# Chriz122/ultralytics_pro

Measured on AMD Instinct MI355X. Metric: images/sec (whole job = n_gpus x per-GPU bs=32) YOLOv8n 640x640 (forward + Detect decode + NMS), higher is better.
Workload: dtype bf16

## Files before the change

### include/upa.h

```cpp
#ifndef UPA_H
#define UPA_H
#include <stddef.h>
#include <stdint.h>

#ifdef __cplusplus
extern "C" {
#endif

enum { UPA_F32 = 0, UPA_BF16 = 1, UPA_U8_BGR_HWC = 2  };
enum { UPA_ACT_NONE = 0, UPA_ACT_SILU = 1, UPA_ACT_RELU = 2 };
enum { UPA_OK = 0, UPA_EINVAL = -1, UPA_EUNSUPPORTED = -2, UPA_EWORKSPACE = -3, UPA_ELAUNCH = -4 };

typedef struct upa_opts {
  uint32_t size;
  int32_t conv_big;
  int32_t conv_big_bm;
  int32_t conv_ckt;
  int32_t no_ws, no_pipe, no_1x1, no_c16, no_upcat;
  int32_t pipe_all;
  int32_t pipe_min_tiles;
  int32_t pipe_wgs, c16_wgs;
  int32_t c1_mt, c1_waves, c1_wgs;
  int32_t pair;
  int32_t pair_tile64, pair_tile32;
  int32_t no_pair_cv2;
  int32_t c2f;
  int32_t c2f16_waves;
  int32_t c2f32_th;
  int32_t no_branch_tail;
  int32_t branch_tail_bm;
  int32_t stem_wgs, stemf_wgs, stemf_waves, stem_no_mfma;
  int32_t ablate_conv, ablate_pipe, ablate_c1, ablate_stem;
  int32_t c2f64_max_px;
  int32_t conv_ws3;
  int32_t no_group;
  int32_t no_c2f32_up;
  int32_t no_xcd;
  int32_t keys_only;
  int32_t conv_p8;
  int32_t c2f_stream;
  int32_t c2f_stream_rows;
  int32_t no_stack_first;
  int32_t no_epi_stats;
  int32_t nms_stages;
  int32_t nms_first_prefix;
  int32_t detect_stream;
  int32_t detect_stream_rows;
  int32_t no_sppf_front;
  int32_t no_c2f16_down;
} upa_opts;

int upa_version(void);
const char* upa_last_error(void);
size_t upa_opts_size(void);

size_t upa_conv_packed_weight_bytes(int cout, int cin, int k, int dtype);
int upa_pack_conv_weight(const float* w_oihw, int cout, int cin, int k, int dtype, void* out);
int upa_conv2d_bias_act(const void* x, int n, int h, int w, int cin, int ldx,
                        const void* w_packed, const float* bias ,
                        void* y, int cout, int ldy,
                        const void* residual , int ldr,
                        int k, int stride, int pad, int act, int dtype, const upa_opts* opts, void* stream);
typedef struct upa_conv_problem {
  const void* x; int32_t n, h, w, cin, ldx;
  const void* w_packed; const float* bias;
  void* y; int32_t cout, ldy;
  const void* residual; int32_t ldr;
} upa_conv_problem;
int upa_conv2d_bias_act_group(const upa_conv_problem* probs, int count, int k, int stride, int pad, int act, int dtype,
                              const upa_opts* opts, void* stream);

int upa_conv2d_pool2(const void* x, int n, int h, int w, int cin, int ldx, const void* w_packed, const float* bias, void* y, int cout,
                     int ldy, int k, int stride, int pad, int act, int dtype, const upa_opts* opts, void* stream);
int upa_conv2d_stem_nchw_pool2(const void* x_nchw, int x_dtype, int n, int cin, int h, int w, const float* w_oihw, const float* bias,
                               void* y, int cout, int ldy, int k, int stride, int pad, int act, int dtype, const upa_opts* opts,
                               void* stream);

int upa_conv_variant(int n, int h, int w, int cin, int cout, int k, int stride, int pad, int dtype, const upa_opts* opts);

int upa_bottleneck_pair(const void* x, int n, int h, int w, int c, int ldx, const void* w1_packed, const float* b1,
                        const void* w2_packed, const float* b2, void* y, int ldy, int residual, int act, int dtype,
                        const upa_opts* opts, void* stream);
int upa_bottleneck_pair_e(const void* x, int n, int h, int w, int c, int cmid, int ldx, const void* w1_packed, const float* b1,
                          const void* w2_packed, const float* b2, void* y, int ldy, int residual, int act, int dtype,
                          const upa_opts* opts, void* stream);


size_t upa_stem_packed_weight_bytes(int cout, int cin, int k);
int upa_pack_stem_weight(const float* w_oihw, int cout, int cin, int k, float* out );
int upa_conv2d_stem_nchw(const void* x_nchw, int x_dtype, int n, int cin, int h, int w,
                         const float* w_oihw, const float* bias, void* y, int cout, int ldy,
                         int k, int stride, int pad, int act, int dtype, const upa_opts* opts, void* stream);

int upa_stem_conv_fused(const void* x, int n, int h, int w, const float* w0, const float* b0, const void* w1,
                        const float* b1, void* y, int ldy, const upa_opts* opts, void* stream);
int upa_stem_conv_fused_k(const void* x, int n, int h, int w, int k0, const float* w0, const float* b0, const void* w1,
                          const float* b1, void* y, int ldy, const upa_opts* opts, void* stream);
int upa_stem_conv_fused_c(const void* x, int n, int h, int w, int k0, int c0, const float* w0, const float* b0, const void* w1,
                          const float* b1, void* y, int ldy, const upa_opts* opts, void* stream);
int upa_stem_conv_fused_s(const void* x, int n, int h, int w, int k0, int s0, int c0, const float* w0, const float* b0,
                          const void* w1, const float* b1, void* y, int ldy, const upa_opts* opts, void* stream);

int upa_maxpool2d(const void* x, int n, int h, int w, int c, int ldx, void* y, int oh, int ow, int ldy,
                  int k, int stride, int pad, int pad_br, int dtype, void* stream);
int upa_sppf_pool3(const void* x, int n, int h, int w, int c, int ldx, void* y1, void* y2, void* y3, int ldy,
                   int dtype, void* stream);
int upa_sppf_front(const void* x, int n, int h, int w, int c1, int ldx, const void* w_packed, const float* bias, void* y, int c_, int ldy, int dtype,
                   const upa_opts* opts, void* stream);
int upa_upsample2x(const void* x, int n, int h, int w, int c, int ldx, void* y, int ldy, int dtype, void* stream);
int upa_copy_view(const void* x, int n, int h, int w, int c, int ldx, void* y, int ldy, int dtype, void* stream);
int upa_copy_to_host(const void* src_dev, void* dst_pinned, size_t bytes, void* stream);
int upa_results_to_host(const void* rows_dev, const int* counts_dev, int batch, int max_rows, int row_bytes,
                        void* rows_pinned, int* counts_pinned, void* stream);
int upa_add_view(const void* a, int lda, const void* b, int ldb, void* y, int ldy, int n, int h, int w, int c,
                 int dtype, void* stream);
int upa_nchw_to_nhwc(const float* x, int n, int c, int h, int w, void* y, int ldy, int dtype, void* stream);
int upa_nhwc_to_nchw(const void* x, int n, int h, int w, int c, int ldx, float* y, int dtype, void* stream);
int upa_letterbox_u8(const void* src, int n, int h0, int w0, long src_image_stride, int src_row_stride, void* dst, int H, int W,
                     int new_h, int new_w, int top, int left, int pad_value, void* stream);


int upa_detect_decode(const void* box, int ldb, const void* cls, int ldc, int n, int h, int w, int reg_max, int nc,
                      float stride_px, float* y, int a_total, int a0, int dtype, void* stream);
int upa_detect_tail(const void* x, int n, int h, int w, int cin, int ldx, const void* w_packed, const float* bias, int cout,
                    int kind, int nc, float stride_px, float* y, int a_total, int a0, void* raw, int ldraw,
                    unsigned long long* best_keys, int dtype, const upa_opts* opts, void* stream);

int upa_conv1x1_upcat(const void* x, int n, int h, int w, int cin, int ldx, const void* up, int up_c, int up_ld,
                      const void* w_packed, const float* bias, void* y, int cout, int ldy, int act, int dtype,
                      const upa_opts* opts, void* stream);

int upa_bottleneck_pair_cv2(const void* x, const void* y0, int n, int h, int w, int ldx, const void* w1_packed, const float* b1,
                            const void* w2_packed, const float* b2, int residual, const void* wc_std, const void* wc_b,
                            const float* bc, void* out, int ldout, int act, int dtype, const upa_opts* opts, void* stream);

int upa_c2f_fused(const void* x, int n, int h, int w, int c1, int ldx, int c, int nb, int shortcut, const void* w1,
                  const float* b1, const void* const* wm, const float* const* bm, const void* w2, const float* b2, void* y,
                  int c2, int ldy, int act, int dtype, const upa_opts* opts, void* stream);

int upa_c2f16_down_fused(const void* x, int n, int h, int w, int ldx, const void* w1, const float* b1, const void* const* wm,
                         const float* const* bm, const void* w2, const float* b2, const void* wd, const float* bd, void* y, int ldy,
                         int dtype, const upa_opts* opts, void* stream);

int upa_c2f64_fused(const void* x, int n, int h, int w, int c1, int ldx, const void* up, int up_c, int up_ld, int nb, int shortcut,
                    const void* w1, const float* b1, const void* const* wm, const float* const* bm, const void* w2,
                    const float* b2, void* y, int c2, int ldy, int act, int dtype, const upa_opts* opts, void* stream);
int upa_c2f32_up_fused(const void* x, int n, int h, int w, int c1, int ldx, const void* up, int up_c, int up_ld, int nb, int shortcut,
                       const void* w1, const float* b1, const void* const* wm, const float* const* bm, const void* w2, const float* b2,
                       void* y, int c2, int ldy, int act, int dtype, const upa_opts* opts, void* stream);

size_t upa_tail_packed_weight_bytes(int cout, int cin);
int upa_pack_tail_weight(const float* w, int cout, int cin, void* out);
int upa_detect_branch_tail(const void* x, int n, int h, int w, int c, int ldx, const void* w3_packed, const float* b3,
                           const void* wt_packed, const float* bt, int kind, int nc, float stride_px, float* y, int a_total,
                           int a0, unsigned long long* best_keys, int dtype, const upa_opts* opts, void* stream);
typedef struct upa_branch_level {
  const void* x; int32_t n, h, w, c, ldx;
  const void* w3_packed; const float* b3;
  const void* wt_packed; const float* bt;
  float stride_px; int32_t a0;
} upa_branch_level;
int upa_detect_branch_tail_group(const upa_branch_level* levels, int count, int kind, int nc, float* y, int a_total,
                                 unsigned long long* best_keys, int dtype, const upa_opts* opts, void* stream);
int upa_detect_head_tails(const upa_branch_level* box, const upa_branch_level* cls, int count, int nc, float* y, int a_total,
                          unsigned long long* best_keys, int dtype, const upa_opts* opts, void* stream);
typedef struct upa_detect_branch {
  int32_t c, reserved;
  const void* w1; const float* b1;
  const void* w2; const float* b2;
  const void* wt; const float* bt;
} upa_detect_branch;
int upa_detect_level_stream(const void* x, int n, int h, int w, int cin, int ldx, const upa_detect_branch* box,
                            const upa_detect_branch* cls, int nc, float stride_px, float* y, int a_total, int a0,
                            unsigned long long* best_keys, int dtype, const upa_opts* opts, void* stream);


size_t upa_nms_workspace_bytes(int b, int nc, int a, int multi_label, int max_nms);
int upa_nms_batched_hot(const float* pred, int b, int nc, int a, float conf_thres, float iou_thres, int multi_label,
                        int agnostic, const uint8_t* classes_mask, int max_det, int max_nms, float max_wh, float* out,
                        int32_t* counts, int32_t* keep_idx, void* workspace, size_t workspace_bytes,
                        const unsigned long long* best_keys, void* stream);
int upa_nms_batched_opts(const float* pred, int b, int nc, int a, float conf_thres, float iou_thres, int multi_label,
                         int agnostic, const uint8_t* classes_mask, int max_det, int max_nms, float max_wh, float* out,
                         int32_t* counts, int32_t* keep_idx, void* workspace, size_t workspace_bytes, const upa_opts* opts,
                         void* stream);
int upa_nms_batched(const float* pred, int b, int nc, int a, float conf_thres, float iou_thres, int multi_label,
                    int agnostic, const uint8_t* classes_mask, int max_det, int max_nms, float max_wh,
                    float* out, int32_t* counts, int32_t* keep_idx, void* workspace, size_t workspace_bytes,
                    void* stream);

int upa_mhsa(const void* q, const void* k, const void* v, int ldqkv, int n, int hw, int heads, int d, float scale,
             const void* residual, int ldr, void* y, int ldy, int dtype, void* stream);

int upa_dwconv2d(const void* x, int n, int h, int w, int c, int ldx, const float* weight, const float* bias, void* y, int ldy, int k,
                 int stride, int pad, int act, int dtype, void* stream);
int upa_psa_attention(const void* qkv, int ldqkv, int n, int h, int w, int heads, int key_dim, int head_dim, float scale,
                      const float* pe_weight, const float* pe_bias, void* y, int ldy, int dtype, void* stream);

int upa_linear(const float* x, long m, int k, int ldx, const void* w_packed, const float* bias, float* y, int n, int ldy,
               const float* residual, int ldr, int act, void* stream);
int upa_linear_bf16(const float* x, long m, int k, int ldx, const void* w_packed, const float* bias, float* y, int n,
                    int ldy, const float* residual, int ldr, int act, void* stream);
int upa_linear_mixed(const void* x, int x_dtype, long m, int k, int ldx, const void* w_packed, const float* bias, void* y,
                     int y_dtype, int n, int ldy, const float* residual, int ldr, int act, void* stream);
int upa_layer_norm(const float* x, const float* residual, int m, int c, const float* gamma, const float* beta, float eps,
                   float* y, void* stream);
int upa_rows_add(const float* a, const float* b, float* y, long m, int c, void* stream);
int upa_rows_scale(const float* x, const float* row_scale, float* y, long m, int c, void* stream);
int upa_rows_gather(const float* x, const int32_t* row_idx, float* y, long m_out, int c, void* stream);
int upa_topk_tokens(const float* scores, int nc, int n_levels, const int32_t* level_hw, int b, int k, int32_t* out_rows,
                    int32_t* out_tok, void* stream);
int upa_box_refine(const float* delta, const float* ref, float* y, long n_boxes, void* stream);
int upa_box_add_anchors(const float* delta, const int32_t* tok, const float* anchors, float* y, long n_boxes, void* stream);
int upa_sigmoid(const float* x, float* y, long n, void* stream);
int upa_rtdetr_output(const float* boxes, const float* scores, float* y, long m, int nc, void* stream);
int upa_rtdetr_postprocess(const float* preds, int b, int q, int nc, float conf, const unsigned char* classes_mask, int max_det,
                           const float* orig_wh, float ow, float oh, float* out, int32_t* counts, void* stream);
int upa_msdeform_attn(const float* value, const int32_t* shapes_hw, int n_levels, int b, int heads, int d,
                      const float* offsets, const float* attn_logits, const float* ref_boxes, int len_q, int n_points,
                      float* y, void* stream);
int upa_msdeform_attn_strided(const void* value, int value_dtype, int ldv, const int32_t* shapes_hw, int n_levels, int b, int heads,
                              int d, const float* offsets, const float* attn_logits, const float* ref_boxes, int len_q,
                              int n_points, float* y, void* stream);


int upa_box_iou(const float* box1, int n, const float* box2, int m, float eps, float* out, void* stream);

int upa_scale_boxes(float* rows, long n, int row_stride, float gain, float pad_x, float pad_y, int padding, float w0,
                    float h0, void* stream);
int upa_match_predictions(const float* det, const int* counts, int b, int max_det, const float* gt, const int* ngt, int max_gt,
                          const float* iou_thresholds, int n_thr, unsigned char* tp, void* stream);


int upa_pack_conv_weight_dev(const float* w_oihw, int cout, int cin, int k, int dtype, int transpose_flip, void* out,
                             void* stream);
typedef struct UpaPackDesc {
  const float* w_oihw;
  void* out;
  int cout, cin, k, dtype, transpose_flip, reserved;
} UpaPackDesc;
int upa_pack_conv_weights_batched(const UpaPackDesc* descs_dev, int n, void* stream);
size_t upa_channel_reduce_workspace_bytes(int c);
int upa_bn_stats(const void* z, long npix, int c, int ldz, double* ws, int dtype, void* stream);
int upa_bn_finalize(const double* ws, long npix, int c, float momentum, float* mean, float* var, float* running_mean,
                    float* running_var, void* stream);
int upa_conv2d_bn_stats(const void* x, int n, int h, int w, int cin, int ldx, const void* w_packed, void* z, int cout, int ldz, int k,
                        int stride, int pad, float momentum, float* mean, float* var, float* running_mean, float* running_var,
                        double* ws, int dtype, const upa_opts* opts, void* stream);
int upa_conv2d_bn_act_fwd(const void* x, int n, int h, int w, int cin, int ldx, const void* w_packed, void* z, int cout, int ldz, int k,
                          int stride, int pad, float momentum, float* mean, float* var, float* running_mean, float* running_var,
                          const float* gamma, const float* beta, float eps, int act, void* y, int ldy, const void* residual, int ldr,
                          double* ws, int dtype, const upa_opts* opts, void* stream);
int upa_bn_act_fwd(const void* z, long npix, int c, int ldz, const float* mean, const float* var, const float* gamma,
                   const float* beta, float eps, int act, void* y, int ldy, const void* residual, int ldr, int dtype,
                   void* stream);
int upa_bn_act_bwd(const void* z, const void* dy, long npix, int c, int ldz, int lddy, const float* mean, const float* var,
                   const float* gamma, const float* beta, float eps, int act, void* dz, int lddz, float* dgamma, float* dbeta,
                   int accumulate, double* ws, int dtype, void* stream);
int upa_conv_bn_act_bwd(const void* x, int n, int h, int w, int cin, int ldx, const void* z, const void* dy, int cout, int ldz, int lddy,
                        const float* mean, const float* var, const float* gamma, const float* beta, float eps, int act, void* dz,
                        int lddz, float* dgamma, float* dbeta, double* ws, float* dw_oihw, void* wgrad_ws, size_t wgrad_ws_bytes,
                        void* side_stream, const void* w_packed_t, void* dx, int lddx, int accumulate_dx, int k, int pad, int dtype,
                        const upa_opts* opts, void* stream);
int upa_channel_sum(const void* z, long npix, int c, int ldz, float* out, int accumulate, double* ws, int dtype, void* stream);
size_t upa_conv2d_wgrad_workspace_bytes(int cin, int cout, int k);
int upa_conv2d_wgrad(const void* x, int n, int h, int w, int cin, int ldx, const void* dz, int cout, int lddz, float* dw_oihw,
                     int k, int stride, int pad, int accumulate, int dtype, void* workspace, size_t workspace_bytes, void* stream);
int upa_conv2d_dgrad_s2(const void* dz, int n, int oh, int ow, int cout, int lddz, const void* phase_w_packed, void* dx, int h, int w,
                        int cin, int lddx, int accumulate, int dtype, const upa_opts* opts, void* stream);
int upa_dilate2x(const void* src, int n, int oh, int ow, int c, int lds, void* dst, int h, int w, int ldd, int dtype,
                 void* stream);
int upa_dgrad_s2_phase_weights(const float* w_oihw, int cout, int cin, float* v, void* stream);
int upa_interleave2x(const void* t00, const void* t01, const void* t10, const void* t11, int n, int oh1, int ow1, int c, int ldt,
                     void* dx, int h, int w, int lddx, int accumulate, int dtype, void* stream);
int upa_upsample2x_bwd(const void* dy, int n, int h, int w, int c, int lddy, void* dx, int lddx, int accumulate, int dtype,
                       void* stream);
size_t upa_maxpool2d_bwd_workspace_bytes(int n, int h, int w, int c, int k, int stride, int pad);
int upa_maxpool2d_bwd(const void* x, const void* dy, int n, int h, int w, int c, int ldx, int lddy, int k, int stride, int pad,
                      void* dx, int lddx, int accumulate, int dtype, void* workspace, size_t workspace_bytes, void* stream);
size_t upa_sumsq_workspace_bytes(void);
int upa_sumsq(const float* g, long n, double* out, int accumulate, void* workspace, void* stream);
int upa_sgd_nesterov_ema(float* p, float* g, float* momentum_buf, float* ema, long n, const double* grad_sumsq, float max_norm,
                         float lr, float momentum, float weight_decay, int first_step, float ema_d, const float* ema_d_dev,
                         int zero_grad, void* stream);
int upa_sgd_nesterov_ema_scaled(float* p, float* g, float* momentum_buf, float* ema, long n, const double* grad_sumsq, float max_norm,
                                float lr, float momentum, float weight_decay, int first_step, float ema_d, const float* ema_d_dev,
                                int zero_grad, const float* scaler_state, void* stream);
int upa_grad_scaler_update(float* scaler_state, const double* grad_sumsq, float growth_factor, float backoff_factor,
                           int growth_interval, void* stream);
int upa_ema_update(float* ema, const float* v, long n, float d, const float* d_dev, void* stream);
int upa_cast_view(const void* src, int src_dtype, int lds, void* dst, int dst_dtype, int ldd, long npix, int c, void* stream);
size_t upa_detection_loss_workspace_bytes(int b, int n_anchors, int max_gt);
int upa_detection_loss(const float* const* feats, float* const* grads, const int* hs, const int* ws, const int* lds,
                       const float* strides, int n_levels, int b, int nc, int reg_max, const float* gt, const int* n_gt,
                       int max_gt, float gain_box, float gain_cls, float gain_dfl, float grad_scale, float* loss_items,
                       void* workspace, size_t workspace_bytes, void* stream);
int upa_detection_loss_scaled(const float* const* feats, float* const* grads, const int* hs, const int* ws, const int* lds,
                              const float* strides, int n_levels, int b, int nc, int reg_max, const float* gt, const int* n_gt,
                              int max_gt, float gain_box, float gain_cls, float gain_dfl, float grad_scale,
                              const float* grad_scale_dev, float* loss_items, void* workspace, size_t workspace_bytes, void* stream);

size_t upa_conv_transpose2x2_packed_weight_bytes(int cin, int cout, int dtype);
int upa_pack_conv_transpose2x2_weight(const float* w, int cin, int cout, int dtype, void* out);
int upa_conv_transpose2x2(const void* x, int n, int h, int w, int cin, int ldx, const void* w_packed, const float* bias, void* y,
                          int cout, int ldy, int dtype, void* stream);
int upa_mask_coef_rows(const void* x, int n, int h, int w, int c, int ldx, int dtype, float* out, int c_total, int c0, int a_total,
                       int a0, void* stream);
int upa_nms_gather_extra(const float* extra, int b, int ne, int a, const int32_t* keep, const int32_t* counts, int max_det,
                         const float* det, float* out, int ldo, void* stream);
int upa_process_mask(const void* protos, int b, int mh, int mw, int nm, int ldp, int dtype, const float* coef, int coef_ld,
                     const float* det, int det_ld, int max_det, const int32_t* counts, int out_h, int out_w, int mode,
                     float crop_sx, float crop_sy, int top, int left, int bottom, int right, unsigned char* masks,
                     int32_t* nonempty, int capacity, int32_t* total, void* stream);

int upa_crop_mask(const float* masks, int n, int h, int w, const float* boxes, int box_ld, float* out, void* stream);
int upa_resize_bilinear(const float* x, int planes, int h, int w, int top, int left, int bottom, int right, float* y, int out_h,
                        int out_w, void* stream);
int upa_copy_rows(const float* src, long rows, int cols, long lds, float* dst, long ldd, void* stream);

int upa_graph_begin(void* stream);
int upa_graph_end(void* stream, void** graph_exec_out);
int upa_graph_launch(void* graph_exec, void* stream);
int upa_graph_destroy(void* graph_exec);

#ifdef __cplusplus
}
#endif
#endif
```

### ultralytics_pro_amd/_lib.py

```python

from __future__ import annotations

import ctypes as C
import os
from pathlib import Path

import torch

UPA_F32, UPA_BF16, UPA_U8_BGR_HWC = 0, 1, 2
UPA_EUNSUPPORTED = -2
ACT_NONE, ACT_SILU, ACT_RELU = 0, 1, 2

_PKG = Path(__file__).resolve().parent
LIB_PATH = Path(os.environ.get("UPA_HIP_LIB", _PKG / "libupa_hip.so"))

_vp, _i, _f, _sz = C.c_void_p, C.c_int, C.c_float, C.c_size_t


class Opts(C.Structure):

    _fields_ = [("size", C.c_uint32), ("conv_big", _i), ("conv_big_bm", _i), ("conv_ckt", _i),
                ("no_ws", _i), ("no_pipe", _i), ("no_1x1", _i), ("no_c16", _i), ("no_upcat", _i),
                ("pipe_all", _i), ("pipe_min_tiles", _i), ("pipe_wgs", _i), ("c16_wgs", _i),
                ("c1_mt", _i), ("c1_waves", _i), ("c1_wgs", _i),
                ("pair", _i), ("pair_tile64", _i), ("pair_tile32", _i), ("no_pair_cv2", _i),
                ("c2f", _i), ("c2f16_waves", _i), ("c2f32_th", _i),
                ("no_branch_tail", _i), ("branch_tail_bm", _i),
                ("stem_wgs", _i), ("stemf_wgs", _i), ("stemf_waves", _i), ("stem_no_mfma", _i),
                ("ablate_conv", _i), ("ablate_pipe", _i), ("ablate_c1", _i), ("ablate_stem", _i), ("c2f64_max_px", _i), ("conv_ws3", _i), ("no_group", _i), ("no_c2f32_up", _i), ("no_xcd", _i), ("keys_only", _i), ("conv_p8", _i), ("c2f_stream", _i), ("c2f_stream_rows", _i), ("no_stack_first", _i), ("no_epi_stats", _i), ("nms_stages", _i), ("nms_first_prefix", _i), ("detect_stream", _i), ("detect_stream_rows", _i), ("no_sppf_front", _i), ("no_c2f16_down", _i)]

    def __init__(self, **kw):
        super().__init__()
        self.size = C.sizeof(Opts)
        for k, v in kw.items():
            if k in dict(self._fields_):
                setattr(self, k, int(v))
            else:
                raise AttributeError(f"upa_opts has no field '{k}'")

    def replace(self, **kw) -> "Opts":
        o = Opts()
        C.memmove(C.byref(o), C.byref(self), C.sizeof(Opts))
        for k, v in kw.items():
            setattr(o, k, int(v))
        return o

    _ENV = {"UPA_CONV_BIG": ("conv_big", lambda v: {0: 1, 1: 0, 2: 2}[int(v)]), "UPA_CONV_BIG_BM": ("conv_big_bm", int), "UPA_CONV_WS3": ("conv_ws3", int),
            "UPA_CONV_CKT": ("conv_ckt", int), "UPA_CONV_NO_WS": ("no_ws", lambda v: 1), "UPA_CONV_NO_PIPE": ("no_pipe", lambda v: 1),
            "UPA_CONV_NO_1X1": ("no_1x1", lambda v: 1), "UPA_CONV_NO_C16": ("no_c16", lambda v: 1), "UPA_NO_UPCAT": ("no_upcat", lambda v: 1),
            "UPA_PIPE_ALL": ("pipe_all", lambda v: 1), "UPA_PIPE_MIN_TILES": ("pipe_min_tiles", int), "UPA_PIPE_WGS": ("pipe_wgs", int),
            "UPA_C16_WGS": ("c16_wgs", int), "UPA_C1_MT": ("c1_mt", int), "UPA_C1_WAVES": ("c1_waves", int), "UPA_C1_WGS": ("c1_wgs", int),
            "UPA_NO_PAIR": ("pair", lambda v: {0: 2, 1: 1, 2: 0, 3: 3}[int(v)]), "UPA_PAIR_T64": ("pair_tile64", int),
            "UPA_PAIR_T32": ("pair_tile32", int), "UPA_NO_PAIR_CV2": ("no_pair_cv2", int), "UPA_NO_C2F": ("c2f", int),
            "UPA_C2F16_WAVES": ("c2f16_waves", int), "UPA_C2F32_TH": ("c2f32_th", int), "UPA_NO_BRANCH_TAIL": ("no_branch_tail", int),
            "UPA_BRANCH_TAIL_BM": ("branch_tail_bm", int), "UPA_STEM_WGS": ("stem_wgs", int), "UPA_STEMF_WGS": ("stemf_wgs", int),
            "UPA_STEMF_WAVES": ("stemf_waves", int), "UPA_STEM_NO_MFMA": ("stem_no_mfma", lambda v: 1),
            "UPA_CONV_ABLATE": ("ablate_conv", int), "UPA_PIPE_ABLATE": ("ablate_pipe", int), "UPA_C1_ABLATE": ("ablate_c1", int),
            "UPA_STEM_ABLATE": ("ablate_stem", int)}

    @classmethod
    def from_env(cls, env=None) -> "Opts":
        env = os.environ if env is None else env
        o = cls()
        for name, (field, conv) in cls._ENV.items():
            if name in env:
                setattr(o, field, conv(env[name]))
        return o


class BranchLevel(C.Structure):
    _fields_ = [("x", C.c_void_p), ("n", _i), ("h", _i), ("w", _i), ("c", _i), ("ldx", _i), ("w3_packed", C.c_void_p), ("b3", C.c_void_p),
                ("wt_packed", C.c_void_p), ("bt", C.c_void_p), ("stride_px", C.c_float), ("a0", _i)]


class DetectBranch(C.Structure):
    _fields_ = [("c", _i), ("reserved", _i), ("w1", C.c_void_p), ("b1", C.c_void_p), ("w2", C.c_void_p), ("b2", C.c_void_p),
                ("wt", C.c_void_p), ("bt", C.c_void_p)]


class ConvProblem(C.Structure):
    _fields_ = [("x", C.c_void_p), ("n", _i), ("h", _i), ("w", _i), ("cin", _i), ("ldx", _i), ("w_packed", C.c_void_p), ("bias", C.c_void_p),
                ("y", C.c_void_p), ("cout", _i), ("ldy", _i), ("residual", C.c_void_p), ("ldr", _i)]


_op = C.POINTER(Opts)

PROTOTYPES = {
    "upa_version": (_i, []),
    "upa_last_error": (C.c_char_p, []),
    "upa_opts_size": (_sz, []),
    "upa_conv_packed_weight_bytes": (_sz, [_i, _i, _i, _i]),
    "upa_pack_conv_weight": (_i, [_vp, _i, _i, _i, _i, _vp]),
    "upa_conv2d_bias_act": (_i, [_vp, _i, _i, _i, _i, _i, _vp, _vp, _vp, _i, _i, _vp, _i, _i, _i, _i, _i, _i, _op, _vp]),
    "upa_conv_variant": (_i, [_i, _i, _i, _i, _i, _i, _i, _i, _i, _op]),
    "upa_bottleneck_pair": (_i, [_vp, _i, _i, _i, _i, _i, _vp, _vp, _vp, _vp, _vp, _i, _i, _i, _i, _op, _vp]),
    "upa_bottleneck_pair_e": (_i, [_vp, _i, _i, _i, _i, _i, _i, _vp, _vp, _vp, _vp, _vp, _i, _i, _i, _i, _op, _vp]),
    "upa_stem_packed_weight_bytes": (_sz, [_i, _i, _i]),
    "upa_pack_stem_weight": (_i, [_vp, _i, _i, _i, _vp]),
    "upa_conv2d_stem_nchw": (_i, [_vp, _i, _i, _i, _i, _i, _vp, _vp, _vp, _i, _i, _i, _i, _i, _i, _i, _op, _vp]),
    "upa_conv2d_stem_nchw_pool2": (_i, [_vp, _i, _i, _i, _i, _i, _vp, _vp, _vp, _i, _i, _i, _i, _i, _i, _i, _op, _vp]),
    "upa_conv2d_pool2": (_i, [_vp, _i, _i, _i, _i, _i, _vp, _vp, _vp, _i, _i, _i, _i, _i, _i, _i, _op, _vp]),
    "upa_stem_conv_fused": (_i, [_vp, _i, _i, _i, _vp, _vp, _vp, _vp, _vp, _i, _op, _vp]),
    "upa_stem_conv_fused_k": (_i, [_vp, _i, _i, _i, _i, _vp, _vp, _vp, _vp, _vp, _i, _op, _vp]),
    "upa_stem_conv_fused_c": (_i, [_vp, _i, _i, _i, _i, _i, _vp, _vp, _vp, _vp, _vp, _i, _op, _vp]),
    "upa_stem_conv_fused_s": (_i, [_vp, _i, _i, _i, _i, _i, _i, _vp, _vp, _vp, _vp, _vp, _i, _op, _vp]),
    "upa_maxpool2d": (_i, [_vp, _i, _i, _i, _i, _i, _vp, _i, _i, _i, _i, _i, _i, _i, _i, _vp]),
    "upa_sppf_pool3": (_i, [_vp, _i, _i, _i, _i, _i, _vp, _vp, _vp, _i, _i, _vp]),
    "upa_upsample2x": (_i, [_vp, _i, _i, _i, _i, _i, _vp, _i, _i, _vp]),
    "upa_copy_view": (_i, [_vp, _i, _i, _i, _i, _i, _vp, _i, _i, _vp]),
    "upa_copy_to_host": (_i, [_vp, _vp, _sz, _vp]),
    "upa_results_to_host": (_i, [_vp, _vp, _i, _i, _i, _vp, _vp, _vp]),
    "upa_add_view": (_i, [_vp, _i, _vp, _i, _vp, _i, _i, _i, _i, _i, _i, _vp]),
    "upa_nchw_to_nhwc": (_i, [_vp, _i, _i, _i, _i, _vp, _i, _i, _vp]),
    "upa_nhwc_to_nchw": (_i, [_vp, _i, _i, _i, _i, _i, _vp, _i, _vp]),
    "upa_letterbox_u8": (_i, [_vp, _i, _i, _i, C.c_long, _i, _vp, _i, _i, _i, _i, _i, _i, _i, _vp]),
    "upa_detect_decode": (_i, [_vp, _i, _vp, _i, _i, _i, _i, _i, _i, _f, _vp, _i, _i, _i, _vp]),
    "upa_detect_branch_tail_group": (_i, [_vp, _i, _i, _i, _vp, _i, _vp, _i, _op, _vp]),
    "upa_detect_head_tails": (_i, [_vp, _vp, _i, _i, _vp, _i, _vp, _i, _op, _vp]),
    "upa_conv2d_bias_act_group": (_i, [_vp, _i, _i, _i, _i, _i, _i, _op, _vp]),
    "upa_detect_level_stream": (_i, [_vp, _i, _i, _i, _i, _i, _vp, _vp, _i, _f, _vp, _i, _i, _vp, _i, _op, _vp]),
    "upa_detect_tail": (_i, [_vp, _i, _i, _i, _i, _i, _vp, _vp, _i, _i, _i, _f, _vp, _i, _i, _vp, _i, _vp, _i, _op, _vp]),
    "upa_conv1x1_upcat": (_i, [_vp, _i, _i, _i, _i, _i, _vp, _i, _i, _vp, _vp, _vp, _i, _i, _i, _i, _op, _vp]),
    "upa_bottleneck_pair_cv2": (_i, [_vp, _vp, _i, _i, _i, _i, _vp, _vp, _vp, _vp, _i, _vp, _vp, _vp, _vp, _i, _i, _i, _op, _vp]),
    "upa_sppf_front": (_i, [_vp, _i, _i, _i, _i, _i, _vp, _vp, _vp, _i, _i, _i, _op, _vp]),
    "upa_c2f16_down_fused": (_i, [_vp, _i, _i, _i, _i, _vp, _vp, _vp, _vp, _vp, _vp, _vp, _vp, _vp, _i, _i, _op, _vp]),
    "upa_c2f_fused": (_i, [_vp, _i, _i, _i, _i, _i, _i, _i, _i, _vp, _vp, _vp, _vp, _vp, _vp, _vp, _i, _i, _i, _i, _op, _vp]),
    "upa_c2f64_fused": (_i, [_vp, _i, _i, _i, _i, _i, _vp, _i, _i, _i, _i, _vp, _vp, _vp, _vp, _vp, _vp, _vp, _i, _i, _i, _i, _op, _vp]),
    "upa_c2f32_up_fused": (_i, [_vp, _i, _i, _i, _i, _i, _vp, _i, _i, _i, _i, _vp, _vp, _vp, _vp, _vp, _vp, _vp, _i, _i, _i, _i, _op, _vp]),
    "upa_tail_packed_weight_bytes": (_sz, [_i, _i]),
    "upa_pack_tail_weight": (_i, [_vp, _i, _i, _vp]),
    "upa_detect_branch_tail": (_i, [_vp, _i, _i, _i, _i, _i, _vp, _vp, _vp, _vp, _i, _i, _f, _vp, _i, _i, _vp, _i, _op, _vp]),
    "upa_nms_batched_hot": (_i, [_vp, _i, _i, _i, _f, _f, _i, _i, _vp, _i, _i, _f, _vp, _vp, _vp, _vp, _sz, _vp, _vp]),
    "upa_nms_workspace_bytes": (_sz, [_i, _i, _i, _i, _i]),
    "upa_nms_batched": (_i, [_vp, _i, _i, _i, _f, _f, _i, _i, _vp, _i, _i, _f, _vp, _vp, _vp, _vp, _sz, _vp]),
    "upa_nms_batched_opts": (_i, [_vp, _i, _i, _i, _f, _f, _i, _i, _vp, _i, _i, _f, _vp, _vp, _vp, _vp, _sz, _vp, _vp]),
    "upa_mhsa": (_i, [_vp, _vp, _vp, _i, _i, _i, _i, _i, _f, _vp, _i, _vp, _i, _i, _vp]),
    "upa_dwconv2d": (_i, [_vp, _i, _i, _i, _i, _i, _vp, _vp, _vp, _i, _i, _i, _i, _i, _i, _vp]),
    "upa_psa_attention": (_i, [_vp, _i, _i, _i, _i, _i, _i, _i, _f, _vp, _vp, _vp, _i, _i, _vp]),
    "upa_linear": (_i, [_vp, C.c_long, _i, _i, _vp, _vp, _vp, _i, _i, _vp, _i, _i, _vp]),
    "upa_linear_bf16": (_i, [_vp, C.c_long, _i, _i, _vp, _vp, _vp, _i, _i, _vp, _i, _i, _vp]),
    "upa_linear_mixed": (_i, [_vp, _i, C.c_long, _i, _i, _vp, _vp, _vp, _i, _i, _i, _vp, _i, _i, _vp]),
    "upa_layer_norm": (_i, [_vp, _vp, _i, _i, _vp, _vp, _f, _vp, _vp]),
    "upa_rows_add": (_i, [_vp, _vp, _vp, C.c_long, _i, _vp]),
    "upa_rows_scale": (_i, [_vp, _vp, _vp, C.c_long, _i, _vp]),
    "upa_rows_gather": (_i, [_vp, _vp, _vp, C.c_long, _i, _vp]),
    "upa_topk_tokens": (_i, [_vp, _i, _i, _vp, _i, _i, _vp, _vp, _vp]),
    "upa_box_refine": (_i, [_vp, _vp, _vp, C.c_long, _vp]),
    "upa_box_add_anchors": (_i, [_vp, _vp, _vp, _vp, C.c_long, _vp]),
    "upa_sigmoid": (_i, [_vp, _vp, C.c_long, _vp]),
    "upa_rtdetr_output": (_i, [_vp, _vp, _vp, C.c_long, _i, _vp]),
    "upa_rtdetr_postprocess": (_i, [_vp, _i, _i, _i, _f, _vp, _i, _vp, _f, _f, _vp, _vp, _vp]),
    "upa_msdeform_attn": (_i, [_vp, _vp, _i, _i, _i, _i, _vp, _vp, _vp, _i, _i, _vp, _vp]),
    "upa_msdeform_attn_strided": (_i, [_vp, _i, _i, _vp, _i, _i, _i, _i, _vp, _vp, _vp, _i, _i, _vp, _vp]),
    "upa_box_iou": (_i, [_vp, _i, _vp, _i, _f, _vp, _vp]),
    "upa_match_predictions": (_i, [_vp, _vp, _i, _i, _vp, _vp, _i, _vp, _i, _vp, _vp]),
    "upa_scale_boxes": (_i, [_vp, C.c_long, _i, _f, _f, _f, _i, _f, _f, _vp]),
    "upa_pack_conv_weight_dev": (_i, [_vp, _i, _i, _i, _i, _i, _vp, _vp]),
    "upa_channel_reduce_workspace_bytes": (_sz, [_i]),
    "upa_bn_stats": (_i, [_vp, C.c_long, _i, _i, _vp, _i, _vp]),
    "upa_bn_finalize": (_i, [_vp, C.c_long, _i, _f, _vp, _vp, _vp, _vp, _vp]),
    "upa_conv2d_bn_act_fwd": (_i, [_vp, _i, _i, _i, _i, _i, _vp, _vp, _i, _i, _i, _i, _i, _f, _vp, _vp, _vp, _vp, _vp, _vp, _f, _i, _vp, _i, _vp, _i,
                                    _vp, _i, _vp, _vp]),
    "upa_conv2d_bn_stats": (_i, [_vp, _i, _i, _i, _i, _i, _vp, _vp, _i, _i, _i, _i, _i, _f, _vp, _vp, _vp, _vp, _vp, _i, _vp, _vp]),
    "upa_bn_act_fwd": (_i, [_vp, C.c_long, _i, _i, _vp, _vp, _vp, _vp, _f, _i, _vp, _i, _vp, _i, _i, _vp]),
    "upa_bn_act_bwd": (_i, [_vp, _vp, C.c_long, _i, _i, _i, _vp, _vp, _vp, _vp, _f, _i, _vp, _i, _vp, _vp, _i, _vp, _i, _vp]),
    "upa_conv_bn_act_bwd": (_i, [_vp, _i, _i, _i, _i, _i, _vp, _vp, _i, _i, _i, _vp, _vp, _vp, _vp, _f, _i, _vp, _i, _vp, _vp, _vp, _vp, _vp, _sz,
                                  _vp, _vp, _vp, _i, _i, _i, _i, _i, _vp, _vp]),
    "upa_conv2d_dgrad_s2": (_i, [_vp, _i, _i, _i, _i, _i, _vp, _vp, _i, _i, _i, _i, _i, _i, _vp, _vp]),
    "upa_channel_sum": (_i, [_vp, C.c_long, _i, _i, _vp, _i, _vp, _i, _vp]),
    "upa_conv2d_wgrad_workspace_bytes": (_sz, [_i, _i, _i]),
    "upa_conv2d_wgrad": (_i, [_vp, _i, _i, _i, _i, _i, _vp, _i, _i, _vp, _i, _i, _i, _i, _i, _vp, _sz, _vp]),
    "upa_dilate2x": (_i, [_vp, _i, _i, _i, _i, _i, _vp, _i, _i, _i, _i, _vp]),
    "upa_dgrad_s2_phase_weights": (_i, [_vp, _i, _i, _vp, _vp]),
    "upa_interleave2x": (_i, [_vp, _vp, _vp, _vp, _i, _i, _i, _i, _i, _vp, _i, _i, _i, _i, _i, _vp]),
    "upa_upsample2x_bwd": (_i, [_vp, _i, _i, _i, _i, _i, _vp, _i, _i, _i, _vp]),
    "upa_maxpool2d_bwd_workspace_bytes": (_sz, [_i, _i, _i, _i, _i, _i, _i]),
    "upa_maxpool2d_bwd": (_i, [_vp, _vp, _i, _i, _i, _i, _i, _i, _i, _i, _i, _vp, _i, _i, _i, _vp, _sz, _vp]),
    "upa_pack_conv_weights_batched": (_i, [_vp, _i, _vp]),
    "upa_sumsq_workspace_bytes": (C.c_size_t, []),
    "upa_sumsq": (_i, [_vp, C.c_long, _vp, _i, _vp, _vp]),
    "upa_sgd_nesterov_ema": (_i, [_vp, _vp, _vp, _vp, C.c_long, _vp, _f, _f, _f, _f, _i, _f, _vp, _i, _vp]),
    "upa_ema_update": (_i, [_vp, _vp, C.c_long, _f, _vp, _vp]),
    "upa_cast_view": (_i, [_vp, _i, _i, _vp, _i, _i, C.c_long, _i, _vp]),
    "upa_detection_loss_workspace_bytes": (_sz, [_i, _i, _i]),
    "upa_detection_loss": (_i, [_vp, _vp, _vp, _vp, _vp, _vp, _i, _i, _i, _i, _vp, _vp, _i, _f, _f, _f, _f, _vp, _vp, _sz, _vp]),
    "upa_detection_loss_scaled": (_i, [_vp, _vp, _vp, _vp, _vp, _vp, _i, _i, _i, _i, _vp, _vp, _i, _f, _f, _f, _f, _vp, _vp, _vp, _sz, _vp]),
    "upa_sgd_nesterov_ema_scaled": (_i, [_vp, _vp, _vp, _vp, C.c_long, _vp, _f, _f, _f, _f, _i, _f, _vp, _i, _vp, _vp]),
    "upa_grad_scaler_update": (_i, [_vp, _vp, _f, _f, _i, _vp]),
    "upa_conv_transpose2x2_packed_weight_bytes": (_sz, [_i, _i, _i]),
    "upa_pack_conv_transpose2x2_weight": (_i, [_vp, _i, _i, _i, _vp]),
    "upa_conv_transpose2x2": (_i, [_vp, _i, _i, _i, _i, _i, _vp, _vp, _vp, _i, _i, _i, _vp]),
    "upa_mask_coef_rows": (_i, [_vp, _i, _i, _i, _i, _i, _i, _vp, _i, _i, _i, _i, _vp]),
    "upa_nms_gather_extra": (_i, [_vp, _i, _i, _i, _vp, _vp, _i, _vp, _vp, _i, _vp]),
    "upa_process_mask": (_i, [_vp, _i, _i, _i, _i, _i, _i, _vp, _i, _vp, _i, _i, _vp, _i, _i, _i, _f, _f, _i, _i, _i, _i, _vp, _vp, _i,
                              _vp, _vp]),
    "upa_crop_mask": (_i, [_vp, _i, _i, _i, _vp, _i, _vp, _vp]),
    "upa_resize_bilinear": (_i, [_vp, _i, _i, _i, _i, _i, _i, _i, _vp, _i, _i, _vp]),
    "upa_copy_rows": (_i, [_vp, C.c_long, _i, C.c_long, _vp, C.c_long, _vp]),
    "upa_graph_begin": (_i, [_vp]),
    "upa_graph_end": (_i, [_vp, C.POINTER(_vp)]),
    "upa_graph_launch": (_i, [_vp, _vp]),
    "upa_graph_destroy": (_i, [_vp]),
}

_lib = None


class UpaError(RuntimeError):
    pass


def lib() -> C.CDLL:
    global _lib
    if _lib is None:
        if not LIB_PATH.is_file():
            raise UpaError(
                f"{LIB_PATH} not found: build it with `python -c 'import __graft_entry__ as g; g.build()'` "
                "(make -C ultralytics_pro_amd/csrc). The HIP path has no fallback.")
        handle = C.CDLL(str(LIB_PATH))
        for name, (res, args) in PROTOTYPES.items():
            fn = getattr(handle, name)
            fn.restype, fn.argtypes = res, args
        if handle.upa_opts_size() != C.sizeof(Opts):
            raise UpaError(f"{LIB_PATH}: upa_opts is {handle.upa_opts_size()} bytes, the binding's mirror {C.sizeof(Opts)} - rebuild the library")
        _lib = handle
    return _lib


def check(rc: int, what: str = "") -> None:
    if rc != 0:
        msg = lib().upa_last_error().decode(errors="replace")
        raise UpaError(f"{what or 'upa call'} failed (rc={rc}): {msg}")


def dtype_code(dt: torch.dtype) -> int:
    if dt == torch.float32:
        return UPA_F32
    if dt == torch.bfloat16:
        return UPA_BF16
    raise UpaError(f"unsupported activation dtype {dt}; use torch.float32 (parity) or torch.bfloat16 (perf)")


def current_stream(device=None) -> int:
    return torch.cuda.current_stream(device).cuda_stream


def require_gpu(t: torch.Tensor, what: str) -> None:
    if not t.is_cuda:
        raise UpaError(f"{what}: tensor is on {t.device}; the HIP path only runs on an MI355X (cuda:N) - "
                       "there is deliberately no CPU fallback")
```

### ultralytics_pro_amd/csrc/conv_big.hip

```cpp
#include <stdlib.h>

#include <mutex>
#include <type_traits>
#include <unordered_map>

#include "common.h"
#include "conv_pipe.h"
UPA_STAMP_DEFINE(conv_big)

template <int KS, int STRIDE, int WM, int WN, int MT, int NT, int TAIL = 0>
__device__ __forceinline__ void conv_big_body(const BigParams& p, const int bid0) {
  static_assert(WM * WN == 8, "8 waves per workgroup");
  static_assert(TAIL == 0 || TAIL == 3 || TAIL == 4 || WN == 1, "a tail needs every channel of a pixel in one wave");
  static_assert(TAIL != 1 || (NT % 2) == 0, "box branch: 64 channels");
  static_assert(TAIL != 3 || (NT % 2) == 0, "the statistics epilogue pairs n-tiles");
  static_assert(TAIL != 4 || ((NT % 2) == 0 && KS == 2 && STRIDE == 1), "the interleaving epilogue: 2 x 2 phase kernels, paired n-tiles");
  constexpr int NTB = WN * NT;
  constexpr int WBUF = 2 * NTB * 1024;
  extern __shared__ __attribute__((aligned(16))) char smem[];
  const int tid = threadIdx.x;
  const int lane = tid & 63;
  const int wave = __builtin_amdgcn_readfirstlane(tid >> 6);
  const int r = lane & 15, g = lane >> 4;
  const int wm = wave / WN, wn = wave % WN;

  const int tilesPerImg = p.tilesX * p.tilesY;
  int bid = p.no_xcd ? bid0 : upa_xcd_tile(bid0, tilesPerImg * p.N);
  const int n = bid / tilesPerImg;
  bid -= n * tilesPerImg;
  const int tyi = bid / p.tilesX;
  const int txi = bid - tyi * p.tilesX;
  const int oy0 = tyi * p.TH, ox0 = txi * p.TW;
  const int iy0 = oy0 * STRIDE - p.pad, ix0 = ox0 * STRIDE - p.pad;
  const int ntb0 = blockIdx.y * NTB;

  const int haloItems = p.IH * p.IWp * 8;
  const int haloPadded = (haloItems + 63) & ~63;
  char* hal = smem;
  char* wbuf = smem + (size_t)haloPadded * 16;

  int pl0[MT], pty[MT], ptx[MT];
#pragma unroll
  for (int i = 0; i < MT; ++i) {
    const int pp = (wm * MT + i) * 16 + r;
    int ty = (int)__umulhi((unsigned)pp, p.magicTW);
    int tx = pp - ty * p.TW;
    if (ty >= p.TH) { ty = p.TH; tx = 0; }
    pty[i] = ty;
    ptx[i] = tx;
    pl0[i] = ty < p.TH ? (ty * STRIDE) * p.IWp + tx : 0;
  }

  f32x4 acc[MT][NT];
#pragma unroll
  for (int i = 0; i < MT; ++i)
#pragma unroll
    for (int j = 0; j < NT; ++j) acc[i][j] = f32x4{0.f, 0.f, 0.f, 0.f};

  constexpr int TAPS = KS * KS;
  const int nChunks = (p.KTT + 1) >> 1;

  auto stage_halo = [&](int c) __attribute__((always_inline)) {
    const int c0 = c * 64;
    for (int base = wave * 64; base < haloPadded; base += 512) {
      const int idx = base + lane;
      const int pix = idx >> 3;
      const int slot = idx & 7;
      const int cg = slot ^ (pix & 7);
      const int py = (int)__umulhi((unsigned)pix, p.magicIW);
      const int qx = pix - py * p.IWp;
      int px = qx;
      if constexpr (STRIDE == 2) px = qx < p.HALF ? 2 * qx : 2 * (qx - p.HALF) + 1;
      const int iy = iy0 + py, ix = ix0 + px;
      const int ch = c0 + cg * 8;
      const char* src = reinterpret_cast<const char*>(g_zero16);
      if (idx < haloItems && px < p.IW && iy >= 0 && iy < p.H && ix >= 0 && ix < p.W && ch < p.Cin)
        src = p.x + ((((size_t)n * p.H + iy) * p.W + ix) * (size_t)p.ldx + ch) * 2;
      lds_dma16(src, hal + base * 16);
    }
  };
  auto stage_w = [&](int c, int tap, int b) __attribute__((always_inline)) {
#pragma unroll
    for (int f0 = 0; f0 < 2 * NTB; f0 += 8) {
      const int f = f0 + wave;
      if (f < 2 * NTB) {
        const int kt = f / NTB, j = f - kt * NTB;
        const int ktg = c * 2 + kt;
        const int nt = ntb0 + j;
        const char* src = reinterpret_cast<const char*>(g_zero16);
        if (ktg < p.KTT && nt < p.NTn) src = p.w + (((size_t)(tap * p.KTT + ktg) * p.NTn + nt) * 64 + lane) * 16;
        lds_dma16(src, wbuf + b * WBUF + f * 1024);
      }
    }
  };

  UPA_STAMP_AT(0);
  UPA_STAMP_HWID();
  stage_halo(0);
  stage_w(0, 0, 0);
  int buf = 0;
  for (int c = 0; c < nChunks; ++c) {
    int kh = 0, kw = 0;
#pragma unroll 1
    for (int tap = 0; tap < TAPS; ++tap) {
      asm volatile("s_waitcnt vmcnt(0)" ::: "memory");
      __syncthreads();
      if (c == 0) UPA_STAMP_AT(1 + tap);
      if (tap + 1 < TAPS) stage_w(c, tap + 1, buf ^ 1);
      const int tapshift = kh * p.IWp + (STRIDE == 2 ? (kw >> 1) + (kw & 1) * p.HALF : kw);
      const char* wb = wbuf + buf * WBUF + (wn * NT) * 1024 + lane * 16;
      int paddr[MT], pswz[MT];
#pragma unroll
      for (int i = 0; i < MT; ++i) {
        const int pl = pl0[i] + tapshift;
        paddr[i] = pl * 128;
        pswz[i] = pl & 7;
      }
#pragma unroll
      for (int kt = 0; kt < 2; ++kt) {
        if constexpr (TAIL == 2) {
          if (kt == 1 && c * 2 + 1 >= p.KTT) break;
        }
        if constexpr (NT <= 6) {
          u32x4 a[NT], b[MT];
#pragma unroll
          for (int j = 0; j < NT; ++j) a[j] = *reinterpret_cast<const u32x4*>(wb + (kt * NTB + j) * 1024);
#pragma unroll
          for (int i = 0; i < MT; ++i) b[i] = *reinterpret_cast<const u32x4*>(hal + paddr[i] + (((kt * 4 + g) ^ pswz[i]) << 4));
#pragma unroll
          for (int i = 0; i < MT; ++i)
#pragma unroll
            for (int j = 0; j < NT; ++j)
              acc[i][j] = __builtin_amdgcn_mfma_f32_16x16x32_bf16(*reinterpret_cast<const bf16x8*>(&a[j]),
                                                                  *reinterpret_cast<const bf16x8*>(&b[i]), acc[i][j], 0, 0, 0);
        } else {
          constexpr int GS = (NT + 1) / 2;
          u32x4 b[MT];
#pragma unroll
          for (int i = 0; i < MT; ++i) b[i] = *reinterpret_cast<const u32x4*>(hal + paddr[i] + (((kt * 4 + g) ^ pswz[i]) << 4));
#pragma unroll
          for (int j0 = 0; j0 < NT; j0 += GS) {
            u32x4 a[GS];
#pragma unroll
            for (int j = 0; j < GS; ++j)
              if (j0 + j < NT) a[j] = *reinterpret_cast<const u32x4*>(wb + (kt * NTB + j0 + j) * 1024);
#pragma unroll
            for (int i = 0; i < MT; ++i)
#pragma unroll
              for (int j = 0; j < GS; ++j)
                if (j0 + j < NT)
                  acc[i][j0 + j] = __builtin_amdgcn_mfma_f32_16x16x32_bf16(*reinterpret_cast<const bf16x8*>(&a[j]),
                                                                           *reinterpret_cast<const bf16x8*>(&b[i]), acc[i][j0 + j], 0, 0, 0);
            __builtin_amdgcn_sched_barrier(0);
          }
        }
      }
      buf ^= 1;
      if (++kw == KS) { kw = 0; ++kh; }
    }
    if (c + 1 < nChunks) {
      __syncthreads();
      stage_halo(c + 1);
      stage_w(c + 1, 0, buf);
    }
  }
  UPA_STAMP_AT(10);

  if constexpr (TAIL == 1 || TAIL == 2) {
    f32x4 bv[NT];
#pragma unroll
    for (int j = 0; j < NT; ++j) bv[j] = *reinterpret_cast<const f32x4*>(p.bias + j * 16 + g * 4);
    f32x4 acc2[MT][NT];
#pragma unroll
    for (int i = 0; i < MT; ++i)
#pragma unroll
      for (int j = 0; j < NT; ++j) acc2[i][j] = f32x4{0.f, 0.f, 0.f, 0.f};
#pragma unroll
    for (int s2 = 0; s2 < NT / 2; ++s2) {
      u32x4 hb[MT];
#pragma unroll
      for (int i = 0; i < MT; ++i) {
        float v0[4], v1[4];
#pragma unroll
        for (int q = 0; q < 4; ++q) {
          v0[q] = act_rcp<UPA_ACT_SILU>(acc[i][2 * s2][q] + bv[2 * s2][q]);
          v1[q] = act_rcp<UPA_ACT_SILU>(acc[i][2 * s2 + 1][q] + bv[2 * s2 + 1][q]);
        }
        hb[i] = u32x4{pack_bf16x2(v0[0], v0[1]), pack_bf16x2(v0[2], v0[3]), pack_bf16x2(v1[0], v1[1]), pack_bf16x2(v1[2], v1[3])};
      }
#pragma unroll
      for (int j = 0; j < NT; ++j) {
        const u32x4 a2 = *reinterpret_cast<const u32x4*>(p.tw + ((size_t)(s2 * NT + j) * 64 + lane) * 16);
#pragma unroll
        for (int i = 0; i < MT; ++i)
          acc2[i][j] = __builtin_amdgcn_mfma_f32_16x16x32_bf16(*reinterpret_cast<const bf16x8*>(&a2),
                                                               *reinterpret_cast<const bf16x8*>(&hb[i]), acc2[i][j], 0, 0, 0);
      }
    }
    if constexpr (NT & 1) {
      typedef __attribute__((ext_vector_type(4))) short s16x4;
      constexpr int j0 = NT - 1, s2 = NT / 2;
      u32x2 hh[MT];
#pragma unroll
      for (int i = 0; i < MT; ++i) {
        float v0[4];
#pragma unroll
        for (int q = 0; q < 4; ++q) v0[q] = act_rcp<UPA_ACT_SILU>(acc[i][j0][q] + bv[j0][q]);
        hh[i] = u32x2{pack_bf16x2(v0[0], v0[1]), pack_bf16x2(v0[2], v0[3])};
      }
#pragma unroll
      for (int j = 0; j < NT; ++j) {
        const u32x2 a2 = *reinterpret_cast<const u32x2*>(p.tw + ((size_t)(s2 * NT + j) * 64 + lane) * 16);
#pragma unroll
        for (int i = 0; i < MT; ++i)
          acc2[i][j] = __builtin_amdgcn_mfma_f32_16x16x16bf16_1k(*reinterpret_cast<const s16x4*>(&a2),
                                                                 *reinterpret_cast<const s16x4*>(&hh[i]), acc2[i][j], 0, 0, 0);
      }
    }
    f32x4 tbv[NT];
#pragma unroll
    for (int j = 0; j < NT; ++j) tbv[j] = *reinterpret_cast<const f32x4*>(p.tb + j * 16 + g * 4);
#pragma unroll
    for (int i = 0; i < MT; ++i) {
      const int oy = oy0 + pty[i], ox = ox0 + ptx[i];
      const bool pok = pty[i] < p.TH && oy < p.OH && ox < p.OW;
      const int al = pok ? oy * p.OW + ox : 0;
      if constexpr (TAIL == 1) {
        static_assert(TAIL != 1 || NT == 4, "box branch = 4 sides x 16 bins");
        f32x4 v[4];
#pragma unroll
        for (int j = 0; j < 4; ++j) v[j] = acc2[i][j] + tbv[j];
        upa_detect_box_store(p.de, v, n, al, pok, g);
      } else {
        float best = -1.f;
        int bc = 0;
        if (p.de.keys_only) {
          f32x4 lg[NT];
#pragma unroll
          for (int j = 0; j < NT; ++j) lg[j] = acc2[i][j] + tbv[j];
          upa_detect_cls_keys_only<NT>(p.de, lg, pok, g, best, bc);
        } else {
#pragma unroll
          for (int j = 0; j < NT; ++j) upa_detect_cls_store(p.de, acc2[i][j] + tbv[j], j, n, al, pok, g, best, bc);
        }
        if (p.de.best_keys) upa_detect_best_key_store(p.de, best, bc, n, al, pok, lane);
      }
    }
    return;
  }

  if constexpr (TAIL == 3) {
    const int cw = (blockIdx.y * NTB + wn * NT) * 16;
    float* red = reinterpret_cast<float*>(smem);
    auto row16 = [](float v) __attribute__((always_inline)) {
      v += __uint_as_float(__builtin_amdgcn_update_dpp(0, __float_as_uint(v), 0xB1, 0xF, 0xF, true));
      v += __uint_as_float(__builtin_amdgcn_update_dpp(0, __float_as_uint(v), 0x4E, 0xF, 0xF, true));
      v += __uint_as_float(__builtin_amdgcn_update_dpp(0, __float_as_uint(v), 0x141, 0xF, 0xF, true));
      v += __uint_as_float(__builtin_amdgcn_update_dpp(0, __float_as_uint(v), 0x140, 0xF, 0xF, true));
      return v;
    };
    __syncthreads();
#pragma unroll
    for (int j = 0; j < NT; j += 2) {
      float ss[2][4], sq[2][4];
#pragma unroll
      for (int jj = 0; jj < 2; ++jj)
#pragma unroll
        for (int q = 0; q < 4; ++q) ss[jj][q] = sq[jj][q] = 0.f;
      const int cb = 16 * (j + (g & 1)) + 8 * (g >> 1);
#pragma unroll
      for (int i = 0; i < MT; ++i) {
        const int oy = oy0 + pty[i], ox = ox0 + ptx[i];
        const bool pok = pty[i] < p.TH && oy < p.OH && ox < p.OW;
        const size_t pixoff = ((size_t)n * p.OH + oy) * p.OW + ox;
        const unsigned pk[2][2] = {{pack_bf16x2(acc[i][j][0], acc[i][j][1]), pack_bf16x2(acc[i][j][2], acc[i][j][3])},
                                   {pack_bf16x2(acc[i][j + 1][0], acc[i][j + 1][1]), pack_bf16x2(acc[i][j + 1][2], acc[i][j + 1][3])}};
        const float mk = pok ? 1.f : 0.f;
#pragma unroll
        for (int jj = 0; jj < 2; ++jj)
#pragma unroll
          for (int h2 = 0; h2 < 2; ++h2) {
            const float a = __uint_as_float(pk[jj][h2] << 16) * mk, b = __uint_as_float(pk[jj][h2] & 0xFFFF0000u) * mk;
            ss[jj][2 * h2] += a; sq[jj][2 * h2] = fmaf(a, a, sq[jj][2 * h2]);
            ss[jj][2 * h2 + 1] += b; sq[jj][2 * h2 + 1] = fmaf(b, b, sq[jj][2 * h2 + 1]);
          }
        auto lo = __builtin_amdgcn_permlane16_swap(pk[0][0], pk[1][0], false, false);
        auto hi = __builtin_amdgcn_permlane16_swap(pk[0][1], pk[1][1], false, false);
        if (pok && cw + cb < p.Cout) *reinterpret_cast<u32x4*>(p.y + (pixoff * p.ldy + cw + cb) * 2) = u32x4{lo[0], hi[0], lo[1], hi[1]};
      }
#pragma unroll
      for (int jj = 0; jj < 2; ++jj) {
#pragma unroll
        for (int q = 0; q < 4; ++q) { ss[jj][q] = row16(ss[jj][q]); sq[jj][q] = row16(sq[jj][q]); }
        if (r == 0) {
          *reinterpret_cast<f32x4*>(red + (wave * 2 + 0) * (NT * 16) + (j + jj) * 16 + 4 * g) = f32x4{ss[jj][0], ss[jj][1], ss[jj][2], ss[jj][3]};
          *reinterpret_cast<f32x4*>(red + (wave * 2 + 1) * (NT * 16) + (j + jj) * 16 + 4 * g) = f32x4{sq[jj][0], sq[jj][1], sq[jj][2], sq[jj][3]};
        }
      }
    }
    __syncthreads();
    if (tid < 2 * NTB * 16) {
      const int k = tid / (NTB * 16), chw = tid - k * (NTB * 16);
      const int wn_ = chw / (NT * 16), cl = chw - wn_ * (NT * 16);
      float t = 0.f;
#pragma unroll
      for (int m = 0; m < WM; ++m) t += red[((m * WN + wn_) * 2 + k) * (NT * 16) + cl];
      const int ch = blockIdx.y * NTB * 16 + chw;
      if (ch < p.stats_ld) p.stats[((size_t)blockIdx.x * 2 + k) * p.stats_ld + ch] = t;
    }
    return;
  }

  const int cw = (blockIdx.y * NTB + wn * NT) * 16;
  constexpr bool LAZY_BIAS = NT > 6;
  auto bias_of = [&](int j) __attribute__((always_inline)) {
    const int co = cw + j * 16 + g * 4;
    return (p.bias && co < p.Cout) ? *reinterpret_cast<const f32x4*>(p.bias + co) : f32x4{0.f, 0.f, 0.f, 0.f};
  };
  f32x4 biasv[LAZY_BIAS ? 1 : NT];
  if constexpr (!LAZY_BIAS) {
#pragma unroll
    for (int j = 0; j < NT; ++j) biasv[j] = bias_of(j);
  }
  auto epilogue = [&](auto act_tag) __attribute__((always_inline)) {
    constexpr int ACT = decltype(act_tag)::value;
#pragma unroll
    for (int i = 0; i < MT; ++i) {
      const int oy = oy0 + pty[i], ox = ox0 + ptx[i];
      const bool pok = pty[i] < p.TH && oy < p.OH && ox < p.OW;
      const size_t pixoff = ((size_t)n * p.OH + oy) * p.OW + ox;
      char* yrow = p.y + (pixoff * p.ldy + cw) * 2;
      const char* rrow = p.res ? p.res + (pixoff * p.ldr + cw) * 2 : nullptr;
#pragma unroll
      for (int j = 0; j + 1 < NT; j += 2) {
        const int cb = 16 * (j + (g & 1)) + 8 * (g >> 1);
        const f32x4 bj0 = LAZY_BIAS ? bias_of(j) : biasv[LAZY_BIAS ? 0 : j], bj1 = LAZY_BIAS ? bias_of(j + 1) : biasv[LAZY_BIAS ? 0 : j + 1];
        float v0[4], v1[4];
#pragma unroll
        for (int q = 0; q < 4; ++q) {
          v0[q] = act_rcp<ACT>(acc[i][j][q] + bj0[q]);
          v1[q] = act_rcp<ACT>(acc[i][j + 1][q] + bj1[q]);
        }
        bool ok = pok && cw + cb < p.Cout;
        char* dst = yrow + cb * 2;
        const char* rsrc = rrow ? rrow + cb * 2 : nullptr;
        if constexpr (TAIL == 4) {
          const int ch = cw + cb;
          const int ph = ch / p.il_c, c = ch - ph * p.il_c;
          const int y = 2 * (oy - 1) + (ph >> 1), x = 2 * (ox - 1) + (ph & 1);
          ok = ok && y >= 0 && y < p.il_h && x >= 0 && x < p.il_w;
          const size_t off = ((((size_t)n * p.il_h + y) * p.il_w + x) * p.ldy + c) * 2;
          dst = p.y + off;
          rsrc = p.res ? p.res + off : nullptr;
        }
        if (p.res) {
          float x8[8];
#pragma unroll
          for (int q = 0; q < 4; ++q) {
            auto sw = __builtin_amdgcn_permlane16_swap(__float_as_uint(v0[q]), __float_as_uint(v1[q]), false, false);
            x8[q] = __uint_as_float(sw[0]);
            x8[4 + q] = __uint_as_float(sw[1]);
          }
          if (ok) {
            const u32x4 rv = *reinterpret_cast<const u32x4*>(rsrc);
#pragma unroll
            for (int q = 0; q < 4; ++q) {
              x8[2 * q] += __uint_as_float(rv[q] << 16);
              x8[2 * q + 1] += __uint_as_float(rv[q] & 0xFFFF0000u);
            }
            *reinterpret_cast<u32x4*>(dst) = u32x4{pack_bf16x2(x8[0], x8[1]), pack_bf16x2(x8[2], x8[3]),
                                                   pack_bf16x2(x8[4], x8[5]), pack_bf16x2(x8[6], x8[7])};
          }
        } else {
          auto lo = __builtin_amdgcn_permlane16_swap(pack_bf16x2(v0[0], v0[1]), pack_bf16x2(v1[0], v1[1]), false, false);
          auto hi = __builtin_amdgcn_permlane16_swap(pack_bf16x2(v0[2], v0[3]), pack_bf16x2(v1[2], v1[3]), false, false);
          if (ok) *reinterpret_cast<u32x4*>(dst) = u32x4{lo[0], hi[0], lo[1], hi[1]};
        }
      }
      if constexpr (NT & 1) {
        constexpr int j = NT - 1;
        const int cb = 16 * j + 4 * g;
        float v[4];
        const f32x4 bj = LAZY_BIAS ? bias_of(j) : biasv[LAZY_BIAS ? 0 : j];
#pragma unroll
        for (int q = 0; q < 4; ++q) v[q] = act_rcp<ACT>(acc[i][j][q] + bj[q]);
        if (pok && cw + cb < p.Cout) {
          if (p.res) {
            const u32x2 rv = *reinterpret_cast<const u32x2*>(rrow + cb * 2);
            v[0] += __uint_as_float(rv[0] << 16); v[1] += __uint_as_float(rv[0] & 0xFFFF0000u);
            v[2] += __uint_as_float(rv[1] << 16); v[3] += __uint_as_float(rv[1] & 0xFFFF0000u);
          }
          *reinterpret_cast<u32x2*>(yrow + cb * 2) = u32x2{pack_bf16x2(v[0], v[1]), pack_bf16x2(v[2], v[3])};
        }
      }
    }
  };
  if (p.act == UPA_ACT_SILU) epilogue(std::integral_constant<int, UPA_ACT_SILU>{});
  else if (p.act == UPA_ACT_RELU) epilogue(std::integral_constant<int, UPA_ACT_RELU>{});
  else epilogue(std::integral_constant<int, UPA_ACT_NONE>{});
  UPA_STAMP_AT(11);
#ifdef UPA_STAMP
  asm volatile("s_waitcnt vmcnt(0)" ::: "memory");
  UPA_STAMP_AT(12);
#endif
}

template <int KS, int STRIDE, int WM, int WN, int MT, int NT, int TAIL = 0>
__global__ __launch_bounds__(512, 4) void conv_big_kernel(const BigParams p) {
  conv_big_body<KS, STRIDE, WM, WN, MT, NT, TAIL>(p, (int)blockIdx.x);
}

template <int KS, int STRIDE, int WM, int WN, int MT, int NT, int TAIL = 0>
__global__ __launch_bounds__(512, 4) void conv_big_pair_kernel(const BigParams p0, const BigParams p1, const int split) {
  if ((int)blockIdx.x < split) conv_big_body<KS, STRIDE, WM, WN, MT, NT, TAIL>(p0, (int)blockIdx.x);
  else conv_big_body<KS, STRIDE, WM, WN, MT, NT, TAIL>(p1, (int)blockIdx.x - split);
}
template <int KS, int STRIDE, int WM, int WN, int MT, int NT, int TAIL = 0>
__global__ __launch_bounds__(512, 4) void conv_big_tri_kernel(const BigParams p0, const BigParams p1, const BigParams p2, const int s0,
                                                              const int s1) {
  if ((int)blockIdx.x < s0) conv_big_body<KS, STRIDE, WM, WN, MT, NT, TAIL>(p0, (int)blockIdx.x);
  else if ((int)blockIdx.x < s1) conv_big_body<KS, STRIDE, WM, WN, MT, NT, TAIL>(p1, (int)blockIdx.x - s0);
  else conv_big_body<KS, STRIDE, WM, WN, MT, NT, TAIL>(p2, (int)blockIdx.x - s1);
}

template <int KS_, int STRIDE_, int WM_, int WN_, int MT_, int NT_, int TAIL_>
struct BigCfg {
  static constexpr int NTB = WN_ * NT_;
  __device__ static __forceinline__ void run(const BigParams& p, int bid) { conv_big_body<KS_, STRIDE_, WM_, WN_, MT_, NT_, TAIL_>(p, bid); }
};
template <class CA, class CB>
__global__ __launch_bounds__(512, 4) void conv_big_mix_kernel(const BigParams a0, const BigParams a1, const BigParams b0, const BigParams b1,
                                                              const int s0, const int s1, const int s2) {
  const int b = (int)blockIdx.x;
  if (b < s0) CA::run(a0, b);
  else if (b < s1) CA::run(a1, b - s0);
  else if (b < s2) CB::run(b0, b - s1);
  else CB::run(b1, b - s2);
}

namespace {
void big_halo_geometry(BigParams& p, bool tight = false) {
  p.IH = (p.TH - 1) * p.stride + p.KS;
  p.IW = (p.TW - 1) * p.stride + p.KS;
  p.HALF = p.stride == 2 ? (p.IW + 1) / 2 : 0;
  const int minp = p.stride == 2 ? 2 * p.HALF : p.IW;
  p.IWp = tight ? minp : upa_lds_pick_pitch(minp, p.TW, p.TH * p.TW, p.stride);
  p.magicTW = (unsigned)((0x100000000ULL + p.TW - 1) / p.TW);
  p.magicIW = (unsigned)((0x100000000ULL + p.IWp - 1) / p.IWp);
}
size_t big_halo_bytes(const BigParams& p) { return (((size_t)p.IH * p.IWp * 8 + 63) & ~(size_t)63) * 16; }

bool big_pick_tile(BigParams& p, int bm, int ntb, size_t lds_cap) {
  struct Pick { int th, tw, tight; };
  static std::mutex mu;
  static std::unordered_map<unsigned long long, Pick> memo;
  const unsigned long long key = ((unsigned long long)p.OH << 48) ^ ((unsigned long long)p.OW << 32) ^ ((unsigned long long)bm << 20) ^
                                 ((unsigned long long)ntb << 12) ^ ((unsigned long long)(lds_cap >> 9) << 3) ^ ((unsigned long long)p.KS << 56) ^ (p.KS == 3 ? 4u : 0u) ^
                                 (p.stride == 2 ? 2u : 0u);
  {
    std::lock_guard<std::mutex> lk(mu);
    auto it = memo.find(key);
    if (it != memo.end()) {
      if (it->second.th <= 0) return false;
      p.TH = it->second.th; p.TW = it->second.tw;
      big_halo_geometry(p, it->second.tight != 0);
      return true;
    }
  }
  long best = -1;
  int bth = 0, btw = 0;
  bool btight = false;
  for (int tw = 2; tw <= 256 && tw <= ((p.OW + 1) & ~1); ++tw) {
    int th0 = bm / tw;
    if (th0 > p.OH) th0 = p.OH;
    if (th0 < 1) continue;
    const int thb = cdiv(p.OH, cdiv(p.OH, th0));
    for (int pass = 0; pass < 2; ++pass) {
      const int th = pass ? thb : th0;
      if (pass && thb == th0) break;
      for (int tight = 0; tight < 2; ++tight) {
        p.TH = th; p.TW = tw;
        big_halo_geometry(p, tight != 0);
        const size_t lds = big_halo_bytes(p) + 2 * (size_t)(2 * ntb * 1024) + 256;
        if (lds > lds_cap) continue;
        const long tiles = (long)cdiv(p.OW, tw) * cdiv(p.OH, th);
        const long cost = tiles * 65536 + (long)p.IH * p.IWp;
        if (best < 0 || cost < best) { best = cost; bth = th; btw = tw; btight = tight != 0; }
        break;
      }
    }
  }
  p.TH = bth; p.TW = btw;
  if (best >= 0) big_halo_geometry(p, btight);
  {
    std::lock_guard<std::mutex> lk(mu);
    memo[key] = Pick{best >= 0 ? bth : 0, btw, btight ? 1 : 0};
  }
  return best >= 0;
}

template <int KS, int STRIDE, int WM, int WN, int MT, int NT, int TAIL = 0>
int big_launch_inst(const BigParams& p, size_t lds, hipStream_t s) {
  constexpr int NTB = WN * NT;
  const dim3 grid((unsigned)((long)p.tilesX * p.tilesY * p.N), (unsigned)cdiv(p.NTn, NTB));
  auto kern = conv_big_kernel<KS, STRIDE, WM, WN, MT, NT, TAIL>;
  if (hipError_t e = upa_full_lds<conv_big_kernel<KS, STRIDE, WM, WN, MT, NT, TAIL>>(); e != hipSuccess) {
    upa_set_error("conv_big: cannot raise LDS limit: %s", hipGetErrorString(e));
    return UPA_ELAUNCH;
  }
  hipLaunchKernelGGL(kern, grid, dim3(512), lds, s, p);
  UPA_LAUNCH_CHECK();
  return UPA_OK;
}

template <int KS, int STRIDE, int WM, int WN, int MT, int NT, int TAIL = 0>
int big_launch_pair_inst(const BigParams& p0, const BigParams& p1, size_t lds, hipStream_t s) {
  constexpr int NTB = WN * NT;
  const long t0 = (long)p0.tilesX * p0.tilesY * p0.N, t1 = (long)p1.tilesX * p1.tilesY * p1.N;
  if (cdiv(p0.NTn, NTB) != cdiv(p1.NTn, NTB) || t0 + t1 >= (1L << 31)) return UPA_EUNSUPPORTED;
  const dim3 grid((unsigned)(t0 + t1), (unsigned)cdiv(p0.NTn, NTB));
  if (hipError_t e = upa_full_lds<conv_big_pair_kernel<KS, STRIDE, WM, WN, MT, NT, TAIL>>(); e != hipSuccess) {
    upa_set_error("conv_big: cannot raise LDS limit: %s", hipGetErrorString(e));
    return UPA_ELAUNCH;
  }
  hipLaunchKernelGGL((conv_big_pair_kernel<KS, STRIDE, WM, WN, MT, NT, TAIL>), grid, dim3(512), lds, s, p0, p1, (int)t0);
  UPA_LAUNCH_CHECK();
  return UPA_OK;
}

template <int KS, int STRIDE, int WM, int WN, int MT, int NT, int TAIL = 0>
int big_launch_tri_inst(const BigParams& p0, const BigParams& p1, const BigParams& p2, size_t lds, hipStream_t s) {
  constexpr int NTB = WN * NT;
  const long t0 = (long)p0.tilesX * p0.tilesY * p0.N, t1 = (long)p1.tilesX * p1.tilesY * p1.N, t2 = (long)p2.tilesX * p2.tilesY * p2.N;
  if (cdiv(p0.NTn, NTB) != cdiv(p1.NTn, NTB) || cdiv(p0.NTn, NTB) != cdiv(p2.NTn, NTB) || t0 + t1 + t2 >= (1L << 31)) return UPA_EUNSUPPORTED;
  const dim3 grid((unsigned)(t0 + t1 + t2), (unsigned)cdiv(p0.NTn, NTB));
  if (hipError_t e = upa_full_lds<conv_big_tri_kernel<KS, STRIDE, WM, WN, MT, NT, TAIL>>(); e != hipSuccess) {
    upa_set_error("conv_big: cannot raise LDS limit: %s", hipGetErrorString(e));
    return UPA_ELAUNCH;
  }
  hipLaunchKernelGGL((conv_big_tri_kernel<KS, STRIDE, WM, WN, MT, NT, TAIL>), grid, dim3(512), lds, s, p0, p1, p2, (int)t0, (int)(t0 + t1));
  UPA_LAUNCH_CHECK();
  return UPA_OK;
}

template <class CA, class CB>
int big_launch_mix(const BigParams* pa, int na, const BigParams* pb, int nb, size_t lds, hipStream_t s) {
  long t[4] = {0, 0, 0, 0};
  for (int i = 0; i < na; ++i) { t[i] = (long)pa[i].tilesX * pa[i].tilesY * pa[i].N; if (pa[i].NTn > CA::NTB) return UPA_EUNSUPPORTED; }
  for (int i = 0; i < nb; ++i) { t[2 + i] = (long)pb[i].tilesX * pb[i].tilesY * pb[i].N; if (pb[i].NTn > CB::NTB) return UPA_EUNSUPPORTED; }
  const long tot = t[0] + t[1] + t[2] + t[3];
  if (tot >= (1L << 31)) return UPA_EUNSUPPORTED;
  if (hipError_t e = upa_full_lds<conv_big_mix_kernel<CA, CB>>(); e != hipSuccess) {
    upa_set_error("conv_big: cannot raise LDS limit: %s", hipGetErrorString(e));
    return UPA_ELAUNCH;
  }
  hipLaunchKernelGGL((conv_big_mix_kernel<CA, CB>), dim3((unsigned)tot), dim3(512), lds, s, pa[0], pa[na > 1 ? 1 : 0], pb[0], pb[nb > 1 ? 1 : 0],
                     (int)t[0], (int)(t[0] + t[1]), (int)(t[0] + t[1] + t[2]));
  UPA_LAUNCH_CHECK();
  return UPA_OK;
}

template <int WM, int WN, int MT, int NT>
int big_launch_ks(const BigParams& p, size_t lds, hipStream_t s) {
  if (p.KS == 1) return big_launch_inst<1, 1, WM, WN, MT, NT>(p, lds, s);
  if (p.KS == 2) return big_launch_inst<2, 1, WM, WN, MT, NT>(p, lds, s);
  if (p.stride == 2) return big_launch_inst<3, 2, WM, WN, MT, NT>(p, lds, s);
  return big_launch_inst<3, 1, WM, WN, MT, NT>(p, lds, s);
}
}

extern "C" size_t upa_tail_packed_weight_bytes(int cout, int cin) {
  return (size_t)cdiv(cin, 32) * cdiv(cout, 16) * 1024;
}

static inline unsigned short big_host_bf16(float f) {
  unsigned u;
  memcpy(&u, &f, 4);
  if ((u & 0x7FFFFFFFu) > 0x7F800000u) return (unsigned short)((u >> 16) | 0x40);
  u += 0x7FFFu + ((u >> 16) & 1u);
  return (unsigned short)(u >> 16);
}

extern "C" int upa_pack_tail_weight(const float* w, int cout, int cin, void* out) {
  UPA_CHECK_ARG(w && out && cout > 0 && cin > 0, "pack_tail_weight: bad args");
  const int ks = cdiv(cin, 32), nt = cdiv(cout, 16);
  unsigned short* o = (unsigned short*)out;
  size_t idx = 0;
  for (int s = 0; s < ks; ++s)
    for (int j = 0; j < nt; ++j)
      for (int lane = 0; lane < 64; ++lane) {
        const int g = lane >> 4, r = lane & 15;
        const int co = 16 * j + r;
        for (int e = 0; e < 8; ++e, ++idx) {
          const int ci = 32 * s + (e < 4 ? 4 * g + e : 16 + 4 * g + e - 4);
          o[idx] = big_host_bf16((co < cout && ci < cin) ? w[(size_t)co * cin + ci] : 0.f);
        }
      }
  return UPA_OK;
}

namespace {
int branch_tail_prepare(BigParams& p, int& ntb, int& bm, size_t& lds, const void* x, int n, int h, int w, int c, int ldx,
                        const void* w3_packed, const float* b3, const void* wt_packed, const float* bt, int kind, int nc,
                        float stride_px, float* y, int a_total, int a0, unsigned long long* best_keys, int dtype, const upa_opts* opts) {
  UPA_CHECK_ARG(x && w3_packed && b3 && wt_packed && bt && y, "detect_branch_tail: null pointer");
  UPA_CHECK_ARG(kind == 1 || kind == 2, "detect_branch_tail: kind must be 1 (box) or 2 (class)");
  UPA_CHECK_ARG(n > 0 && h > 0 && w > 0 && a0 >= 0 && a0 + h * w <= a_total, "detect_branch_tail: level does not fit a_total");
  const int off = UPA_OPT(opts, no_branch_tail);
  ntb = kind == 1 ? 4 : (c == 80 ? 5 : 6);
  if (off || dtype != UPA_BF16 || c % 8 != 0 || ldx % 8 != 0 || h * w < 2 || w < 2 || (kind == 1 && c != 64) ||
      (kind == 2 && (c > 96 || nc > ntb * 16)) || ((uintptr_t)x % 16) != 0 || !upa_magic_exact((long)h * w - 1, w)) {
    upa_set_error("detect_branch_tail: outside the fused form (bf16; box c = 64; class c <= 96, nc <= 96)");
    return UPA_EUNSUPPORTED;
  }
  memset(&p, 0, sizeof(p));
  p.x = (const char*)x; p.w = (const char*)w3_packed; p.bias = b3; p.tw = (const char*)wt_packed; p.tb = bt;
  p.N = n; p.H = h; p.W = w; p.Cin = c; p.ldx = ldx; p.OH = h; p.OW = w; p.Cout = ntb * 16; p.KS = 3; p.stride = 1; p.pad = 1;
  p.act = UPA_ACT_SILU;
  p.KTT = cdiv(c, 32);
  p.NTn = ntb;
  p.de.y = y; p.de.a_total = a_total; p.de.a0 = a0; p.de.HW = h * w; p.de.W = w;
  p.de.magicHW = upa_magic_div(h * w); p.de.magicW = upa_magic_div(w);
  p.de.nc = nc; p.de.stride_px = stride_px;
  if (kind == 2 && best_keys && (long)a_total * nc < (1L << 31)) p.de.best_keys = best_keys;
  p.de.keys_only = (p.de.best_keys && UPA_OPT(opts, keys_only)) ? 1 : 0;
  p.no_xcd = UPA_OPT(opts, no_xcd);
  const long px = (long)n * h * w;
  bm = (px + 255) / 256 < upa_num_cus() ? 128 : 256;
  if (const int f = UPA_OPT(opts, branch_tail_bm); f == 128 || f == 256) bm = f;
  if (!big_pick_tile(p, bm, ntb, 80 * 1024 - 512) && !big_pick_tile(p, bm, ntb, 160 * 1024)) return UPA_EUNSUPPORTED;
  p.tilesX = cdiv(p.OW, p.TW);
  p.tilesY = cdiv(p.OH, p.TH);
  lds = big_halo_bytes(p) + 2 * (size_t)(2 * ntb * 1024) + 256;
  return UPA_OK;
}
int branch_tail_launch(const BigParams& p, int kind, int ntb, int bm, size_t lds, hipStream_t s) {
  if (kind == 1) return bm == 256 ? big_launch_inst<3, 1, 8, 1, 2, 4, 1>(p, lds, s) : big_launch_inst<3, 1, 8, 1, 1, 4, 1>(p, lds, s);
  if (ntb == 5) return bm == 256 ? big_launch_inst<3, 1, 8, 1, 2, 5, 2>(p, lds, s) : big_launch_inst<3, 1, 8, 1, 1, 5, 2>(p, lds, s);
  return bm == 256 ? big_launch_inst<3, 1, 8, 1, 2, 6, 2>(p, lds, s) : big_launch_inst<3, 1, 8, 1, 1, 6, 2>(p, lds, s);
}
}

extern "C" int upa_detect_branch_tail(const void* x, int n, int h, int w, int c, int ldx, const void* w3_packed, const float* b3,
                                      const void* wt_packed, const float* bt, int kind, int nc, float stride_px, float* y,
                                      int a_total, int a0, unsigned long long* best_keys, int dtype, const upa_opts* opts,
                                      void* stream) {
  BigParams p;
  int ntb = 0, bm = 0;
  size_t lds = 0;
  if (const int rc = branch_tail_prepare(p, ntb, bm, lds, x, n, h, w, c, ldx, w3_packed, b3, wt_packed, bt, kind, nc, stride_px, y,
                                         a_total, a0, best_keys, dtype, opts); rc != UPA_OK)
    return rc;
  return branch_tail_launch(p, kind, ntb, bm, lds, (hipStream_t)stream);
}

extern "C" int upa_detect_branch_tail_group(const upa_branch_level* levels, int count, int kind, int nc, float* y, int a_total,
                                            unsigned long long* best_keys, int dtype, const upa_opts* opts, void* stream) {
  UPA_CHECK_ARG(levels && count >= 1 && count <= 8, "detect_branch_tail_group: 1..8 levels");
  BigParams ps[8];
  int ntb[8], bm[8];
  size_t lds[8];
  for (int i = 0; i < count; ++i) {
    const upa_branch_level& v = levels[i];
    if (const int rc = branch_tail_prepare(ps[i], ntb[i], bm[i], lds[i], v.x, v.n, v.h, v.w, v.c, v.ldx, v.w3_packed, v.b3, v.wt_packed,
                                           v.bt, kind, nc, v.stride_px, y, a_total, v.a0, best_keys, dtype, opts); rc != UPA_OK)
      return rc;
  }
  hipStream_t s = (hipStream_t)stream;
  const int grouping = UPA_OPT(opts, no_group);
  auto max3 = [](size_t a, size_t b, size_t c) { return a > b ? (a > c ? a : c) : (b > c ? b : c); };
  for (int i = 0; i < count;) {
    if (grouping == 2 && i + 2 < count && ntb[i] == ntb[i + 1] && ntb[i] == ntb[i + 2] && ntb[i] != 6 && bm[i + 1] == 128 && bm[i + 2] == 128) {
      BigParams p0 = ps[i];
      int ntb0 = ntb[i], bm0 = bm[i];
      size_t lds0 = lds[i];
      int rc = UPA_OK;
      if (bm0 != 128) {
        upa_opts o;
        memset(&o, 0, sizeof(o));
        if (opts) memcpy(&o, opts, opts->size < sizeof(o) ? opts->size : sizeof(o));
        o.size = sizeof(o);
        o.branch_tail_bm = 128;
        const upa_branch_level& v = levels[i];
        rc = branch_tail_prepare(p0, ntb0, bm0, lds0, v.x, v.n, v.h, v.w, v.c, v.ldx, v.w3_packed, v.b3, v.wt_packed, v.bt, kind, nc,
                                 v.stride_px, y, a_total, v.a0, best_keys, dtype, &o);
      }
      if (rc == UPA_OK && bm0 == 128) {
        const size_t l3 = max3(lds0, lds[i + 1], lds[i + 2]);
        rc = kind == 1 ? big_launch_tri_inst<3, 1, 8, 1, 1, 4, 1>(p0, ps[i + 1], ps[i + 2], l3, s)
                       : big_launch_tri_inst<3, 1, 8, 1, 1, 5, 2>(p0, ps[i + 1], ps[i + 2], l3, s);
        if (rc == UPA_OK) { i += 3; continue; }
        if (rc != UPA_EUNSUPPORTED) return rc;
      }
    }
    if (grouping != 1 && i + 1 < count && ntb[i] == ntb[i + 1] && bm[i] == 128 && bm[i + 1] == 128 && ntb[i] != 6) {
      const size_t l2 = lds[i] > lds[i + 1] ? lds[i] : lds[i + 1];
      const int rc = kind == 1 ? big_launch_pair_inst<3, 1, 8, 1, 1, 4, 1>(ps[i], ps[i + 1], l2, s)
                               : big_launch_pair_inst<3, 1, 8, 1, 1, 5, 2>(ps[i], ps[i + 1], l2, s);
      if (rc == UPA_OK) { i += 2; continue; }
      if (rc != UPA_EUNSUPPORTED) return rc;
    }
    if (const int rc = branch_tail_launch(ps[i], kind, ntb[i], bm[i], lds[i], s); rc != UPA_OK) return rc;
    ++i;
  }
  return UPA_OK;
}

extern "C" int upa_detect_head_tails(const upa_branch_level* box, const upa_branch_level* cls, int count, int nc, float* y, int a_total,
                                     unsigned long long* best_keys, int dtype, const upa_opts* opts, void* stream) {
  UPA_CHECK_ARG(box && cls && count >= 1 && count <= 8, "detect_head_tails: 1..8 levels");
  BigParams pb[8], pc[8];
  int ntbb[8], bmb[8], ntbc[8], bmc[8];
  size_t ldsb[8], ldsc[8];
  for (int i = 0; i < count; ++i) {
    const upa_branch_level& b = box[i];
    const upa_branch_level& c = cls[i];
    if (const int rc = branch_tail_prepare(pb[i], ntbb[i], bmb[i], ldsb[i], b.x, b.n, b.h, b.w, b.c, b.ldx, b.w3_packed, b.b3, b.wt_packed, b.bt,
                                           1, nc, b.stride_px, y, a_total, b.a0, nullptr, dtype, opts); rc != UPA_OK)
      return rc;
    if (const int rc = branch_tail_prepare(pc[i], ntbc[i], bmc[i], ldsc[i], c.x, c.n, c.h, c.w, c.c, c.ldx, c.w3_packed, c.b3, c.wt_packed, c.bt,
                                           2, nc, c.stride_px, y, a_total, c.a0, best_keys, dtype, opts); rc != UPA_OK)
      return rc;
  }
  hipStream_t s = (hipStream_t)stream;
  const int grouping = UPA_OPT(opts, no_group);
  auto mx = [](size_t a, size_t b) { return a > b ? a : b; };
  using Box128 = BigCfg<3, 1, 8, 1, 1, 4, 1>;
  using Cls128 = BigCfg<3, 1, 8, 1, 1, 5, 2>;
  using Box256 = BigCfg<3, 1, 8, 1, 2, 4, 1>;
  using Cls256 = BigCfg<3, 1, 8, 1, 2, 5, 2>;
  for (int i = 0; i < count;) {
    if (grouping != 1 && ntbc[i] == 5) {
      if (i + 1 < count && ntbc[i + 1] == 5 && bmb[i] == 128 && bmb[i + 1] == 128 && bmc[i] == 128 && bmc[i + 1] == 128) {
        const size_t l = mx(mx(ldsb[i], ldsb[i + 1]), mx(ldsc[i], ldsc[i + 1]));
        const int rc = big_launch_mix<Cls128, Box128>(pc + i, 2, pb + i, 2, l, s);
        if (rc == UPA_OK) { i += 2; continue; }
        if (rc != UPA_EUNSUPPORTED) return rc;
      }
      if (bmb[i] == bmc[i]) {
        const size_t l = mx(ldsb[i], ldsc[i]);
        const int rc = bmb[i] == 128 ? big_launch_mix<Cls128, Box128>(pc + i, 1, pb + i, 1, l, s) : big_launch_mix<Cls256, Box256>(pc + i, 1, pb + i, 1, l, s);
        if (rc == UPA_OK) { ++i; continue; }
        if (rc != UPA_EUNSUPPORTED) return rc;
      }
    }
    if (const int rc = branch_tail_launch(pb[i], 1, ntbb[i], bmb[i], ldsb[i], s); rc != UPA_OK) return rc;
    if (const int rc = branch_tail_launch(pc[i], 2, ntbc[i], bmc[i], ldsc[i], s); rc != UPA_OK) return rc;
    ++i;
  }
  return UPA_OK;
}

bool upa_conv_big_pick_tile(BigParams& p, int bm, int ntb, size_t lds_cap) { return big_pick_tile(p, bm, ntb, lds_cap); }

bool upa_conv_big_eligible(const ConvShape& s, const upa_opts* opts) {
  const int mode = UPA_OPT(opts, conv_big);
  if (mode == 1) return false;
  const int k = s.k, stride = s.stride, cin = s.cin, cout = s.cout;
  if (s.dtype != UPA_BF16 || !((k == 1 && stride == 1) || (k == 2 && stride == 1) || (k == 3 && (stride == 1 || stride == 2))) || s.pad != k / 2) return false;
  if (cin % 8 != 0 || s.ldx % 8 != 0 || cout % 8 != 0 || s.ldy % 8 != 0 || s.ldr % 8 != 0) return false;
  if (s.act != UPA_ACT_SILU && s.act != UPA_ACT_NONE && s.act != UPA_ACT_RELU) return false;
  if (mode == 2) return cout >= 64;
  const int oh = (s.h + 2 * s.pad - k) / stride + 1, ow = (s.w + 2 * s.pad - k) / stride + 1;
  const long px = (long)s.n * oh * ow;
  if (k == 1) {
    if (cout % 128 != 0 || px < 2048) return false;
    if (cout >= 1024 && cin >= 128 && px >= 32 * 1024) return true;
    return cin >= 512 && !upa_conv1x1_eligible(s, opts);
  }
  if (cin < 64 || px < 2048) return false;
  if (cout % 128 == 0) return cin >= 128 || (px >= 8192 && (stride == 2 || px >= 200 * 1024));
  if (px < 8192) return false;
  if (cout == 80 || cout == 96) return stride == 1 && k == 3;
  if (cout == 144) return stride == 1 && k == 3;
  if (cout == 64) return stride == 1;
  return false;
}

namespace {
int big_prepare(BigParams& p, int& ntb, int& bm, size_t& lds, const upa_opts* opts, bool query_only, int force_ntb = 0) {
  p.KTT = (p.Cin + 31) / 32;
  p.NTn = (p.Cout + 15) / 16;
  ntb = p.NTn <= 4 ? 4 : (p.NTn <= 6 ? 6 : 8);
  if (p.NTn == 5 && p.KS == 3 && p.stride == 1) ntb = 5;
  if (p.NTn == 9 && p.KS == 3 && p.stride == 1) ntb = 9;
  if (force_ntb == 5 && p.NTn <= 5 && p.KS == 3 && p.stride == 1) ntb = 5;
  const long px = (long)p.N * p.OH * p.OW;
  if (ntb == 8 && p.NTn % 4 == 0 && (px + 127) / 128 * cdiv(p.NTn, 8) < upa_num_cus()) ntb = 4;
  const int cols = cdiv(p.NTn, ntb);
  bm = 256;
  if ((px + 255) / 256 * cols < upa_num_cus()) bm = 128;
  if (const int f = UPA_OPT(opts, conv_big_bm); f == 128 || f == 256 || (f == 512 && p.KS == 3 && p.stride == 1 && (ntb == 4 || ntb == 5))) bm = f;
  if (query_only) return UPA_OK;
  if (p.KS == 1) {
    p.N = 1; p.H = 1; p.W = (int)px; p.OH = 1; p.OW = (int)px;
    p.TH = 1; p.TW = bm;
    big_halo_geometry(p, true);
  } else if (!big_pick_tile(p, bm, ntb, 80 * 1024 - 512) && !big_pick_tile(p, bm, ntb, 160 * 1024)) {
    return UPA_EUNSUPPORTED;
  }
  p.tilesX = cdiv(p.OW, p.TW);
  p.tilesY = cdiv(p.OH, p.TH);
  lds = big_halo_bytes(p) + 2 * (size_t)(2 * ntb * 1024) + 256;
  if (lds > 160 * 1024) return UPA_EUNSUPPORTED;
  return UPA_OK;
}
template <int WM, int WN, int MT, int NT>
int big_launch_ks_stats(const BigParams& p, size_t lds, hipStream_t s) {
  if (p.KS == 1) return big_launch_inst<1, 1, WM, WN, MT, NT, 3>(p, lds, s);
  if (p.KS != 3) return UPA_EUNSUPPORTED;
  if (p.stride == 2) return big_launch_inst<3, 2, WM, WN, MT, NT, 3>(p, lds, s);
  return big_launch_inst<3, 1, WM, WN, MT, NT, 3>(p, lds, s);
}
int big_dispatch_stats(const BigParams& p, int ntb, int bm, size_t lds, hipStream_t s) {
  if (bm != 128 && bm != 256) return UPA_EUNSUPPORTED;
  if (ntb == 8) return bm == 256 ? big_launch_ks_stats<4, 2, 4, 4>(p, lds, s) : big_launch_ks_stats<4, 2, 2, 4>(p, lds, s);
  if (ntb == 4) return bm == 256 ? big_launch_ks_stats<8, 1, 2, 4>(p, lds, s) : big_launch_ks_stats<4, 2, 2, 2>(p, lds, s);
  return UPA_EUNSUPPORTED;
}
int big_dispatch(const BigParams& p, int ntb, int bm, size_t lds, hipStream_t s) {
  if (bm == 512) return ntb == 5 ? big_launch_inst<3, 1, 8, 1, 4, 5>(p, lds, s) : big_launch_inst<3, 1, 8, 1, 4, 4>(p, lds, s);
  if (ntb == 5) return bm == 256 ? big_launch_inst<3, 1, 8, 1, 2, 5>(p, lds, s) : big_launch_inst<3, 1, 8, 1, 1, 5>(p, lds, s);
  if (ntb == 9) return bm == 256 ? big_launch_inst<3, 1, 8, 1, 2, 9>(p, lds, s) : big_launch_inst<3, 1, 8, 1, 1, 9>(p, lds, s);
  if (ntb == 8) return bm == 256 ? big_launch_ks<4, 2, 4, 4>(p, lds, s) : big_launch_ks<4, 2, 2, 4>(p, lds, s);
  if (ntb == 6) return bm == 256 ? big_launch_ks<4, 2, 4, 3>(p, lds, s) : big_launch_ks<4, 2, 2, 3>(p, lds, s);
  return bm == 256 ? big_launch_ks<8, 1, 2, 4>(p, lds, s) : big_launch_ks<4, 2, 2, 2>(p, lds, s);
}
}

int upa_conv_big_launch(BigParams p, int query_only, int* variant, void* stream, const upa_opts* opts) {
  p.no_xcd = UPA_OPT(opts, no_xcd);
  int ntb = 0, bm = 0;
  size_t lds = 0;
  const int rc = big_prepare(p, ntb, bm, lds, opts, query_only != 0);
  if (variant) *variant = (1 << 23) | (ntb << 4) | (bm >> 7);
  if (query_only || rc != UPA_OK) return rc;
  return big_dispatch(p, ntb, bm, lds, (hipStream_t)stream);
}

int upa_conv_big_launch_interleave(BigParams p, void* stream, const upa_opts* opts) {
  p.no_xcd = UPA_OPT(opts, no_xcd);
  if (p.KS != 2 || p.stride != 1 || p.act != UPA_ACT_NONE || p.bias || p.il_c % 8 != 0 || p.Cout != 4 * p.il_c) return UPA_EUNSUPPORTED;
  int ntb = 0, bm = 0;
  size_t lds = 0;
  if (const int rc = big_prepare(p, ntb, bm, lds, opts, false); rc != UPA_OK) return rc;
  if (ntb != 8 || (bm != 128 && bm != 256)) return UPA_EUNSUPPORTED;
  hipStream_t s = (hipStream_t)stream;
  return bm == 256 ? big_launch_inst<2, 1, 4, 2, 4, 4, 4>(p, lds, s) : big_launch_inst<2, 1, 4, 2, 2, 4, 4>(p, lds, s);
}

int upa_conv_big_launch_stats(BigParams p, int* rows, long max_rows, void* stream, const upa_opts* opts) {
  p.no_xcd = UPA_OPT(opts, no_xcd);
  if (!p.stats || p.res || p.act != UPA_ACT_NONE) return UPA_EUNSUPPORTED;
  int ntb = 0, bm = 0;
  size_t lds = 0;
  if (const int rc = big_prepare(p, ntb, bm, lds, opts, false); rc != UPA_OK) return rc;
  if ((ntb != 8 && ntb != 4) || (bm != 128 && bm != 256)) return UPA_EUNSUPPORTED;
  const long nrows = (long)p.tilesX * p.tilesY * p.N;
  if (nrows > max_rows) return UPA_EUNSUPPORTED;
  p.stats_ld = p.NTn * 16;
  *rows = (int)nrows;
  return big_dispatch_stats(p, ntb, bm, lds, (hipStream_t)stream);
}

int upa_conv_big_launch_group(const BigParams* probs, int count, int* consumed, void* stream, const upa_opts* opts) {
  *consumed = 0;
  if (count < 2) return UPA_EUNSUPPORTED;
  const int grouping = UPA_OPT(opts, no_group);
  if (grouping == 1) return UPA_EUNSUPPORTED;
  if (count >= 4) {
    BigParams q[4];
    int nt4[4], bm4[4];
    size_t l4[4];
    bool ok = true;
    for (int i = 0; i < 4 && ok; ++i) {
      q[i] = probs[i];
      ok = q[i].KS == 3 && q[i].stride == 1 && big_prepare(q[i], nt4[i], bm4[i], l4[i], opts, false) == UPA_OK && bm4[i] == 128;
    }
    if (ok && nt4[0] == 4 && nt4[1] == 4 && nt4[2] == 5 && nt4[3] == 5) {
      size_t l = l4[0];
      for (int i = 1; i < 4; ++i) l = l4[i] > l ? l4[i] : l;
      const bool sw0 = q[1].Cin > q[0].Cin, sw1 = q[3].Cin > q[2].Cin;
      const BigParams a[2] = {sw1 ? q[3] : q[2], sw1 ? q[2] : q[3]}, b[2] = {sw0 ? q[1] : q[0], sw0 ? q[0] : q[1]};
      const int rc = big_launch_mix<BigCfg<3, 1, 8, 1, 1, 5, 0>, BigCfg<3, 1, 4, 2, 2, 2, 0>>(a, 2, b, 2, l, (hipStream_t)stream);
      if (rc == UPA_OK) { *consumed = 4; return UPA_OK; }
      if (rc != UPA_EUNSUPPORTED) return rc;
    }
  }
  BigParams p[3];
  int ntb[3], bm[3];
  size_t lds[3];
  const int m = count >= 3 && grouping == 2 ? 3 : 2;
  for (int i = 0; i < m; ++i) {
    p[i] = probs[i];
    if (p[i].KS != 3 || p[i].stride != 1) return UPA_EUNSUPPORTED;
    if (const int rc = big_prepare(p[i], ntb[i], bm[i], lds[i], opts, false); rc != UPA_OK) return rc;
  }
  hipStream_t s = (hipStream_t)stream;
  auto ok_ntb = [](int v) { return v == 4 || v == 5; };
  if (m == 3 && ntb[0] == ntb[1] && ntb[0] == ntb[2] && ok_ntb(ntb[0]) && bm[1] == 128 && bm[2] == 128) {
    int rc = UPA_OK;
    if (bm[0] != 128) {
      upa_opts o;
      memset(&o, 0, sizeof(o));
      if (opts) memcpy(&o, opts, opts->size < sizeof(o) ? opts->size : sizeof(o));
      o.size = sizeof(o);
      o.conv_big_bm = 128;
      p[0] = probs[0];
      rc = big_prepare(p[0], ntb[0], bm[0], lds[0], &o, false);
    }
    if (rc == UPA_OK && bm[0] == 128 && ntb[0] == ntb[1]) {
      const size_t l3 = lds[0] > lds[1] ? (lds[0] > lds[2] ? lds[0] : lds[2]) : (lds[1] > lds[2] ? lds[1] : lds[2]);
      rc = ntb[0] == 4 ? big_launch_tri_inst<3, 1, 4, 2, 2, 2>(p[0], p[1], p[2], l3, s) : big_launch_tri_inst<3, 1, 8, 1, 1, 5>(p[0], p[1], p[2], l3, s);
      if (rc == UPA_OK) { *consumed = 3; return UPA_OK; }
      if (rc != UPA_EUNSUPPORTED) return rc;
    }
    p[0] = probs[0];
    if (const int rc2 = big_prepare(p[0], ntb[0], bm[0], lds[0], opts, false); rc2 != UPA_OK) return rc2;
  }
  if (ok_ntb(ntb[0]) && ok_ntb(ntb[1]) && bm[0] == bm[1] && (bm[0] == 128 || bm[0] == 256)) {
    if (ntb[0] != ntb[1]) {
      const int lo = ntb[0] < ntb[1] ? 0 : 1;
      p[lo] = probs[lo];
      int bmf = 0;
      if (const int rc = big_prepare(p[lo], ntb[lo], bmf, lds[lo], opts, false, 5); rc != UPA_OK) return rc;
      if (bmf != bm[1 - lo] || ntb[lo] != 5) return UPA_EUNSUPPORTED;
    }
    const size_t l2 = lds[0] > lds[1] ? lds[0] : lds[1];
    int rc;
    if (bm[0] == 128) rc = ntb[0] == 4 ? big_launch_pair_inst<3, 1, 4, 2, 2, 2>(p[0], p[1], l2, s) : big_launch_pair_inst<3, 1, 8, 1, 1, 5>(p[0], p[1], l2, s);
    else rc = ntb[0] == 4 ? big_launch_pair_inst<3, 1, 8, 1, 2, 4>(p[0], p[1], l2, s) : big_launch_pair_inst<3, 1, 8, 1, 2, 5>(p[0], p[1], l2, s);
    if (rc == UPA_OK) { *consumed = 2; return UPA_OK; }
    if (rc != UPA_EUNSUPPORTED) return rc;
  }
  return UPA_EUNSUPPORTED;
}
```

### ultralytics_pro_amd/csrc/conv_pipe.h

```cpp
#pragma once
struct ConvShape {
  int n, h, w, cin, ldx, cout, ldy, ldr, k, stride, pad, act, dtype;
};
struct PipeParams {
  const char* x;
  char* y;
  const char* res;
  const char* w;
  const float* bias;
  int N, H, W, Cin, ldx, Cout, ldy, ldr;
  int KTT, NTn, nt0;
  int tilesX, tilesY, numTiles;
  int act;
  int pool;
#ifdef UPA_ABLATE
  int ablate;
#endif
};
bool upa_conv_pipe_eligible(const ConvShape& s, const upa_opts* opts);
int upa_conv_pipe_launch(PipeParams p, int query_only, int* variant, void* stream, const upa_opts* opts);

#include "detect_epi.h"
struct C1Params {
  const char* x;
  char* y;
  const char* w;
  const float* bias;
  int P;
  int Cin, ldx, Cout, ldy;
  int KTT, NTn, groups;
  int act;
#ifdef UPA_ABLATE
  int ablate;
#endif
  int epi;
  DetectEpi de;
  float* stats;
  int stats_ld;
  const char* up;
  int upKT, up_ld, upH, upW;
  unsigned upMagicW, upMagicH;
};
bool upa_conv1x1_eligible(const ConvShape& s, const upa_opts* opts);
int upa_conv1x1_launch(C1Params p, int n_pixels, int query_only, int* variant, void* stream, const upa_opts* opts);
int upa_conv1x1_launch_stats(C1Params p, int n_pixels, int* rows, long max_rows, void* stream, const upa_opts* opts);

struct BigParams {
  const char* x;
  char* y;
  const char* res;
  const char* w;
  const float* bias;
  int N, H, W, Cin, ldx, OH, OW, Cout, ldy, ldr;
  int KS, stride, pad;
  int TH, TW, tilesX, tilesY, IH, IW;
  int IWp;
  int HALF;
  int KTT, NTn;
  int act;
  unsigned magicTW, magicIW;
  int no_xcd;
  const char* tw;
  const float* tb;
  DetectEpi de;
  float* stats;
  int stats_ld;
  int il_h, il_w, il_c;
};
bool upa_conv_big_eligible(const ConvShape& s, const upa_opts* opts);
int upa_conv_big_launch(BigParams p, int query_only, int* variant, void* stream, const upa_opts* opts);
int upa_conv_big_launch_stats(BigParams p, int* rows, long max_rows, void* stream, const upa_opts* opts);
int upa_conv_big_launch_interleave(BigParams p, void* stream, const upa_opts* opts);
int upa_conv_big_launch_group(const BigParams* probs, int count, int* consumed, void* stream, const upa_opts* opts);

bool upa_conv_big_pick_tile(BigParams& p, int bm, int ntb, size_t lds_cap);

bool upa_conv_p8_eligible(const ConvShape& s, const upa_opts* opts);
int upa_conv_p8_launch(BigParams p, int query_only, int* variant, void* stream, const upa_opts* opts);

bool upa_conv_ws3_eligible(const ConvShape& s, const upa_opts* opts);
int upa_conv_ws3_launch(BigParams p, int query_only, int* variant, void* stream, const upa_opts* opts);
int upa_conv_ws3_launch_stats(BigParams p, int* rows, long max_rows, void* stream, const upa_opts* opts);

struct PairParams {
  const char* x;
  char* y;
  const char* w1;
  const char* w2;
  const float* b1;
  const float* b2;
  int N, H, W, OH, OW, ldx, ldy;
  int TH, TW, tilesX, tilesY;
  int IWp, MWp;
  unsigned magicIW, magicMW, magicTW;
  const char* y0;
  const char* wc_std;
  const char* wc_b;
  const float* bc;
  char* out; int ldout;
};
```

Before: 61240.

## Hoist address math out of conv_big inner loops with cached halo offsets

Adds a new conv_big body that precomputes per-lane halo source offsets once and reuses them across channel chunks. It also keeps weight source pointers that advance by a fixed tap stride, precomputes the B-operand LDS offsets per kw, and splits the tap loop into kh/kw with kw unrolled. The aim is to cut per-tap integer and address arithmetic and the repeated bounds checks in halo staging. The old body stays as a fallback chosen by a host-side loop-form check (large tiles, unaligned IWp, 32-bit offset overflow, or an opt flag). The cached offsets and unrolled loops raise register pressure and add more template instantiations.

```diff
diff --git a/include/upa.h b/include/upa.h
--- a/include/upa.h
+++ b/include/upa.h
@@ -48,6 +48,7 @@
   int32_t detect_stream_rows;
   int32_t no_sppf_front;
   int32_t no_c2f16_down;
+  int32_t conv_big_loop;
 } upa_opts;
 
 int upa_version(void);
@@ -77,6 +78,7 @@
                                void* stream);
 
 int upa_conv_variant(int n, int h, int w, int cin, int cout, int k, int stride, int pad, int dtype, const upa_opts* opts);
+int upa_conv_big_loop_form(int n, int h, int w, int cin, int cout, int k, int stride, const upa_opts* opts);
 
 int upa_bottleneck_pair(const void* x, int n, int h, int w, int c, int ldx, const void* w1_packed, const float* b1,
                         const void* w2_packed, const float* b2, void* y, int ldy, int residual, int act, int dtype,
diff --git a/ultralytics_pro_amd/_lib.py b/ultralytics_pro_amd/_lib.py
--- a/ultralytics_pro_amd/_lib.py
+++ b/ultralytics_pro_amd/_lib.py
@@ -27,7 +27,7 @@
                 ("c2f", _i), ("c2f16_waves", _i), ("c2f32_th", _i),
                 ("no_branch_tail", _i), ("branch_tail_bm", _i),
                 ("stem_wgs", _i), ("stemf_wgs", _i), ("stemf_waves", _i), ("stem_no_mfma", _i),
-                ("ablate_conv", _i), ("ablate_pipe", _i), ("ablate_c1", _i), ("ablate_stem", _i), ("c2f64_max_px", _i), ("conv_ws3", _i), ("no_group", _i), ("no_c2f32_up", _i), ("no_xcd", _i), ("keys_only", _i), ("conv_p8", _i), ("c2f_stream", _i), ("c2f_stream_rows", _i), ("no_stack_first", _i), ("no_epi_stats", _i), ("nms_stages", _i), ("nms_first_prefix", _i), ("detect_stream", _i), ("detect_stream_rows", _i), ("no_sppf_front", _i), ("no_c2f16_down", _i)]
+                ("ablate_conv", _i), ("ablate_pipe", _i), ("ablate_c1", _i), ("ablate_stem", _i), ("c2f64_max_px", _i), ("conv_ws3", _i), ("no_group", _i), ("no_c2f32_up", _i), ("no_xcd", _i), ("keys_only", _i), ("conv_p8", _i), ("c2f_stream", _i), ("c2f_stream_rows", _i), ("no_stack_first", _i), ("no_epi_stats", _i), ("nms_stages", _i), ("nms_first_prefix", _i), ("detect_stream", _i), ("detect_stream_rows", _i), ("no_sppf_front", _i), ("no_c2f16_down", _i), ("conv_big_loop", _i)]
 
     def __init__(self, **kw):
         super().__init__()
@@ -93,6 +93,7 @@
     "upa_pack_conv_weight": (_i, [_vp, _i, _i, _i, _i, _vp]),
     "upa_conv2d_bias_act": (_i, [_vp, _i, _i, _i, _i, _i, _vp, _vp, _vp, _i, _i, _vp, _i, _i, _i, _i, _i, _i, _op, _vp]),
     "upa_conv_variant": (_i, [_i, _i, _i, _i, _i, _i, _i, _i, _i, _op]),
+    "upa_conv_big_loop_form": (_i, [_i, _i, _i, _i, _i, _i, _i, _op]),
     "upa_bottleneck_pair": (_i, [_vp, _i, _i, _i, _i, _i, _vp, _vp, _vp, _vp, _vp, _i, _i, _i, _i, _op, _vp]),
     "upa_bottleneck_pair_e": (_i, [_vp, _i, _i, _i, _i, _i, _i, _vp, _vp, _vp, _vp, _vp, _i, _i, _i, _i, _op, _vp]),
     "upa_stem_packed_weight_bytes": (_sz, [_i, _i, _i]),
diff --git a/ultralytics_pro_amd/csrc/conv_big.hip b/ultralytics_pro_amd/csrc/conv_big.hip
--- a/ultralytics_pro_amd/csrc/conv_big.hip
+++ b/ultralytics_pro_amd/csrc/conv_big.hip
@@ -8,7 +8,9 @@
 #include "conv_pipe.h"
 UPA_STAMP_DEFINE(conv_big)
 
-template <int KS, int STRIDE, int WM, int WN, int MT, int NT, int TAIL = 0>
+constexpr int big_halo_keep(int mt, int nt) { return mt * nt <= 4 ? 12 : (mt * nt <= 10 ? 6 : 0); }
+constexpr bool big_hoisted(int mt, int nt) { return mt * nt <= 12; }
+template <int KS, int STRIDE, int WM, int WN, int MT, int NT, int TAIL = 0, bool OLD = false>
 __device__ __forceinline__ void conv_big_body(const BigParams& p, const int bid0) {
   static_assert(WM * WN == 8, "8 waves per workgroup");
   static_assert(TAIL == 0 || TAIL == 3 || TAIL == 4 || WN == 1, "a tail needs every channel of a pixel in one wave");
@@ -60,108 +62,270 @@
   constexpr int TAPS = KS * KS;
   const int nChunks = (p.KTT + 1) >> 1;
 
-  auto stage_halo = [&](int c) __attribute__((always_inline)) {
-    const int c0 = c * 64;
-    for (int base = wave * 64; base < haloPadded; base += 512) {
-      const int idx = base + lane;
-      const int pix = idx >> 3;
-      const int slot = idx & 7;
-      const int cg = slot ^ (pix & 7);
-      const int py = (int)__umulhi((unsigned)pix, p.magicIW);
-      const int qx = pix - py * p.IWp;
-      int px = qx;
-      if constexpr (STRIDE == 2) px = qx < p.HALF ? 2 * qx : 2 * (qx - p.HALF) + 1;
-      const int iy = iy0 + py, ix = ix0 + px;
-      const int ch = c0 + cg * 8;
-      const char* src = reinterpret_cast<const char*>(g_zero16);
-      if (idx < haloItems && px < p.IW && iy >= 0 && iy < p.H && ix >= 0 && ix < p.W && ch < p.Cin)
-        src = p.x + ((((size_t)n * p.H + iy) * p.W + ix) * (size_t)p.ldx + ch) * 2;
-      lds_dma16(src, hal + base * 16);
-    }
-  };
-  auto stage_w = [&](int c, int tap, int b) __attribute__((always_inline)) {
-#pragma unroll
-    for (int f0 = 0; f0 < 2 * NTB; f0 += 8) {
-      const int f = f0 + wave;
-      if (f < 2 * NTB) {
+  if constexpr (OLD) {
+    auto stage_halo = [&](int c) __attribute__((always_inline)) {
+      const int c0 = c * 64;
+      for (int base = wave * 64; base < haloPadded; base += 512) {
+        const int idx = base + lane;
+        const int pix = idx >> 3;
+        const int slot = idx & 7;
+        const int cg = slot ^ (pix & 7);
+        const int py = (int)__umulhi((unsigned)pix, p.magicIW);
+        const int qx = pix - py * p.IWp;
+        int px = qx;
+        if constexpr (STRIDE == 2) px = qx < p.HALF ? 2 * qx : 2 * (qx - p.HALF) + 1;
+        const int iy = iy0 + py, ix = ix0 + px;
+        const int ch = c0 + cg * 8;
+        const char* src = reinterpret_cast<const char*>(g_zero16);
+        if (idx < haloItems && px < p.IW && iy >= 0 && iy < p.H && ix >= 0 && ix < p.W && ch < p.Cin)
+          src = p.x + ((((size_t)n * p.H + iy) * p.W + ix) * (size_t)p.ldx + ch) * 2;
+        lds_dma16(src, hal + base * 16);
+      }
+    };
+    auto stage_w = [&](int c, int tap, int b) __attribute__((always_inline)) {
+  #pragma unroll
+      for (int f0 = 0; f0 < 2 * NTB; f0 += 8) {
+        const int f = f0 + wave;
+        if (f < 2 * NTB) {
+          const int kt = f / NTB, j = f - kt * NTB;
+          const int ktg = c * 2 + kt;
+          const int nt = ntb0 + j;
+          const char* src = reinterpret_cast<const char*>(g_zero16);
+          if (ktg < p.KTT && nt < p.NTn) src = p.w + (((size_t)(tap * p.KTT + ktg) * p.NTn + nt) * 64 + lane) * 16;
+          lds_dma16(src, wbuf + b * WBUF + f * 1024);
+        }
+      }
+    };
+
+    UPA_STAMP_AT(0);
+    UPA_STAMP_HWID();
+    stage_halo(0);
+    stage_w(0, 0, 0);
+    int buf = 0;
+    for (int c = 0; c < nChunks; ++c) {
+      int kh = 0, kw = 0;
+  #pragma unroll 1
+      for (int tap = 0; tap < TAPS; ++tap) {
+        asm volatile("s_waitcnt vmcnt(0)" ::: "memory");
+        __syncthreads();
+        if (c == 0) UPA_STAMP_AT(1 + tap);
+        if (tap + 1 < TAPS) stage_w(c, tap + 1, buf ^ 1);
+        const int tapshift = kh * p.IWp + (STRIDE == 2 ? (kw >> 1) + (kw & 1) * p.HALF : kw);
+        const char* wb = wbuf + buf * WBUF + (wn * NT) * 1024 + lane * 16;
+        int paddr[MT], pswz[MT];
+  #pragma unroll
+        for (int i = 0; i < MT; ++i) {
+          const int pl = pl0[i] + tapshift;
+          paddr[i] = pl * 128;
+          pswz[i] = pl & 7;
+        }
+  #pragma unroll
+        for (int kt = 0; kt < 2; ++kt) {
+          if constexpr (TAIL == 2) {
+            if (kt == 1 && c * 2 + 1 >= p.KTT) break;
+          }
+          if constexpr (NT <= 6) {
+            u32x4 a[NT], b[MT];
+  #pragma unroll
+            for (int j = 0; j < NT; ++j) a[j] = *reinterpret_cast<const u32x4*>(wb + (kt * NTB + j) * 1024);
+  #pragma unroll
+            for (int i = 0; i < MT; ++i) b[i] = *reinterpret_cast<const u32x4*>(hal + paddr[i] + (((kt * 4 + g) ^ pswz[i]) << 4));
+  #pragma unroll
+            for (int i = 0; i < MT; ++i)
+  #pragma unroll
+              for (int j = 0; j < NT; ++j)
+                acc[i][j] = __builtin_amdgcn_mfma_f32_16x16x32_bf16(*reinterpret_cast<const bf16x8*>(&a[j]),
+                                                                    *reinterpret_cast<const bf16x8*>(&b[i]), acc[i][j], 0, 0, 0);
+          } else {
+            constexpr int GS = (NT + 1) / 2;
+            u32x4 b[MT];
+  #pragma unroll
+            for (int i = 0; i < MT; ++i) b[i] = *reinterpret_cast<const u32x4*>(hal + paddr[i] + (((kt * 4 + g) ^ pswz[i]) << 4));
+  #pragma unroll
+            for (int j0 = 0; j0 < NT; j0 += GS) {
+              u32x4 a[GS];
+  #pragma unroll
+              for (int j = 0; j < GS; ++j)
+                if (j0 + j < NT) a[j] = *reinterpret_cast<const u32x4*>(wb + (kt * NTB + j0 + j) * 1024);
+  #pragma unroll
+              for (int i = 0; i < MT; ++i)
+  #pragma unroll
+                for (int j = 0; j < GS; ++j)
+                  if (j0 + j < NT)
+                    acc[i][j0 + j] = __builtin_amdgcn_mfma_f32_16x16x32_bf16(*reinterpret_cast<const bf16x8*>(&a[j]),
+                                                                             *reinterpret_cast<const bf16x8*>(&b[i]), acc[i][j0 + j], 0, 0, 0);
+              __builtin_amdgcn_sched_barrier(0);
+            }
+          }
+        }
+        buf ^= 1;
+        if (++kw == KS) { kw = 0; ++kh; }
+      }
+      if (c + 1 < nChunks) {
+        __syncthreads();
+        stage_halo(c + 1);
+        stage_w(c + 1, 0, buf);
+      }
+    }
+  } else {
+    constexpr int HK = big_halo_keep(MT, NT);
+    const bool hkeep = HK > 0 && nChunks > 1 && haloPadded <= HK * 512;
+    unsigned hoff[HK > 0 ? HK : 1];
+    const int cgl = (lane & 7) ^ ((lane >> 3) & 7);
+    const unsigned long long xb =
+        (unsigned long long)p.x + (unsigned long long)((((long long)n * p.H + iy0) * p.W + ix0) * (long long)p.ldx * 2);
+    auto stage_halo = [&](int c, bool first) __attribute__((always_inline)) {
+      const int c0 = c * 64;
+      if (!hkeep) {
+        for (int base = wave * 64; base < haloPadded; base += 512) {
+          const int idx = base + lane;
+          const int pix = idx >> 3;
+          const int py = (int)__umulhi((unsigned)pix, p.magicIW);
+          const int qx = pix - py * p.IWp;
+          int px = qx;
+          if constexpr (STRIDE == 2) px = qx < p.HALF ? 2 * qx : 2 * (qx - p.HALF) + 1;
+          const int iy = iy0 + py, ix = ix0 + px;
+          const int ch = c0 + cgl * 8;
+          const char* src = reinterpret_cast<const char*>(g_zero16);
+          if (idx < haloItems && px < p.IW && iy >= 0 && iy < p.H && ix >= 0 && ix < p.W && ch < p.Cin)
+            src = p.x + ((((size_t)n * p.H + iy) * p.W + ix) * (size_t)p.ldx + ch) * 2;
+          lds_dma16(src, hal + base * 16);
+        }
+        return;
+      }
+      const int ch = c0 + cgl * 8;
+      const bool chok = ch < p.Cin;
+#pragma unroll
+      for (int k = 0; k < HK; ++k) {
+        const int base = wave * 64 + k * 512;
+        if (base < haloPadded) {
+          if (first) {
+            const int idx = base + lane;
+            const int pix = idx >> 3;
+            const int py = (int)__umulhi((unsigned)pix, p.magicIW);
+            const int qx = pix - py * p.IWp;
+            int px = qx;
+            if constexpr (STRIDE == 2) px = qx < p.HALF ? 2 * qx : 2 * (qx - p.HALF) + 1;
+            const int iy = iy0 + py, ix = ix0 + px;
+            const bool in = idx < haloItems && px < p.IW && iy >= 0 && iy < p.H && ix >= 0 && ix < p.W;
+            hoff[k] = in ? (unsigned)(py * p.W + px) * (unsigned)p.ldx * 2u : ~0u;
+          }
+          const char* src = reinterpret_cast<const char*>(g_zero16);
+          if (chok && hoff[k] != ~0u) src = reinterpret_cast<const char*>(xb + hoff[k] + (unsigned)(ch * 2));
+          lds_dma16(src, hal + base * 16);
+        }
+      }
+    };
+    constexpr int NS = (2 * NTB + 7) / 8;
+    const char* wsrc[NS];
+    unsigned wstep[NS], wlane[NS];
+    const unsigned tapBytes = (unsigned)(p.KTT * p.NTn) * 1024u;
+    auto setup_w = [&](int c) __attribute__((always_inline)) {
+#pragma unroll
+      for (int s = 0; s < NS; ++s) {
+        const int f = s * 8 + wave;
         const int kt = f / NTB, j = f - kt * NTB;
-        const int ktg = c * 2 + kt;
-        const int nt = ntb0 + j;
-        const char* src = reinterpret_cast<const char*>(g_zero16);
-        if (ktg < p.KTT && nt < p.NTn) src = p.w + (((size_t)(tap * p.KTT + ktg) * p.NTn + nt) * 64 + lane) * 16;
-        lds_dma16(src, wbuf + b * WBUF + f * 1024);
-      }
-    }
-  };
-
-  UPA_STAMP_AT(0);
-  UPA_STAMP_HWID();
-  stage_halo(0);
-  stage_w(0, 0, 0);
-  int buf = 0;
-  for (int c = 0; c < nChunks; ++c) {
-    int kh = 0, kw = 0;
+        const bool ok = f < 2 * NTB && c * 2 + kt < p.KTT && ntb0 + j < p.NTn;
+        wsrc[s] = ok ? p.w + (size_t)((c * 2 + kt) * p.NTn + ntb0 + j) * 1024 : reinterpret_cast<const char*>(g_zero16);
+        wstep[s] = ok ? tapBytes : 0u;
+        wlane[s] = ok ? (unsigned)lane * 16u : 0u;
+      }
+    };
+    const int wdst0 = haloPadded * 16 + wave * 1024;
+    auto issue_w = [&](int bo) __attribute__((always_inline)) {
+#pragma unroll
+      for (int s = 0; s < NS; ++s)
+        if (s * 8 + 7 < 2 * NTB || s * 8 + wave < 2 * NTB) lds_dma16(wsrc[s] + wlane[s], smem + wdst0 + bo + s * 8192);
+    };
+    int boff[MT][KS];
+#pragma unroll
+    for (int i = 0; i < MT; ++i)
+#pragma unroll
+      for (int kw = 0; kw < KS; ++kw) {
+        const int pl = pl0[i] + (STRIDE == 2 ? (kw >> 1) + (kw & 1) * p.HALF : kw);
+        boff[i][kw] = pl * 128 + ((g ^ (pl & 7)) << 4);
+      }
+    const int rowBytes = p.IWp * 128;
+    const int flip = (p.IWp & 4) << 4;
+    const int wl0 = haloPadded * 16 + (wn * NT) * 1024 + lane * 16;
+
+    UPA_STAMP_AT(0);
+    UPA_STAMP_HWID();
+    stage_halo(0, true);
+    setup_w(0);
+    issue_w(0);
+    int cur = 0;
+    for (int c = 0; c < nChunks; ++c) {
+      int rowoff = 0;
+      int f0v = 0, f1v = 64;
 #pragma unroll 1
-    for (int tap = 0; tap < TAPS; ++tap) {
-      asm volatile("s_waitcnt vmcnt(0)" ::: "memory");
-      __syncthreads();
-      if (c == 0) UPA_STAMP_AT(1 + tap);
-      if (tap + 1 < TAPS) stage_w(c, tap + 1, buf ^ 1);
-      const int tapshift = kh * p.IWp + (STRIDE == 2 ? (kw >> 1) + (kw & 1) * p.HALF : kw);
-      const char* wb = wbuf + buf * WBUF + (wn * NT) * 1024 + lane * 16;
-      int paddr[MT], pswz[MT];
-#pragma unroll
-      for (int i = 0; i < MT; ++i) {
-        const int pl = pl0[i] + tapshift;
-        paddr[i] = pl * 128;
-        pswz[i] = pl & 7;
-      }
-#pragma unroll
-      for (int kt = 0; kt < 2; ++kt) {
-        if constexpr (TAIL == 2) {
-          if (kt == 1 && c * 2 + 1 >= p.KTT) break;
-        }
-        if constexpr (NT <= 6) {
-          u32x4 a[NT], b[MT];
-#pragma unroll
-          for (int j = 0; j < NT; ++j) a[j] = *reinterpret_cast<const u32x4*>(wb + (kt * NTB + j) * 1024);
-#pragma unroll
-          for (int i = 0; i < MT; ++i) b[i] = *reinterpret_cast<const u32x4*>(hal + paddr[i] + (((kt * 4 + g) ^ pswz[i]) << 4));
-#pragma unroll
-          for (int i = 0; i < MT; ++i)
-#pragma unroll
-            for (int j = 0; j < NT; ++j)
-              acc[i][j] = __builtin_amdgcn_mfma_f32_16x16x32_bf16(*reinterpret_cast<const bf16x8*>(&a[j]),
-                                                                  *reinterpret_cast<const bf16x8*>(&b[i]), acc[i][j], 0, 0, 0);
-        } else {
-          constexpr int GS = (NT + 1) / 2;
-          u32x4 b[MT];
-#pragma unroll
-          for (int i = 0; i < MT; ++i) b[i] = *reinterpret_cast<const u32x4*>(hal + paddr[i] + (((kt * 4 + g) ^ pswz[i]) << 4));
-#pragma unroll
-          for (int j0 = 0; j0 < NT; j0 += GS) {
-            u32x4 a[GS];
-#pragma unroll
-            for (int j = 0; j < GS; ++j)
-              if (j0 + j < NT) a[j] = *reinterpret_cast<const u32x4*>(wb + (kt * NTB + j0 + j) * 1024);
-#pragma unroll
-            for (int i = 0; i < MT; ++i)
-#pragma unroll
-              for (int j = 0; j < GS; ++j)
-                if (j0 + j < NT)
-                  acc[i][j0 + j] = __builtin_amdgcn_mfma_f32_16x16x32_bf16(*reinterpret_cast<const bf16x8*>(&a[j]),
-                                                                           *reinterpret_cast<const bf16x8*>(&b[i]), acc[i][j0 + j], 0, 0, 0);
-            __builtin_amdgcn_sched_barrier(0);
+      for (int kh = 0; kh < KS; ++kh) {
+#pragma unroll
+        for (int kw = 0; kw < KS; ++kw) {
+          asm volatile("s_waitcnt vmcnt(0)" ::: "memory");
+          __syncthreads();
+          if (c == 0) UPA_STAMP_AT(1 + kh * KS + kw);
+          if (kw + 1 < KS || kh + 1 < KS) {
+#pragma unroll
+            for (int s = 0; s < NS; ++s) wsrc[s] += wstep[s];
+            issue_w(cur ^ WBUF);
           }
-        }
-      }
-      buf ^= 1;
-      if (++kw == KS) { kw = 0; ++kh; }
-    }
-    if (c + 1 < nChunks) {
-      __syncthreads();
-      stage_halo(c + 1);
-      stage_w(c + 1, 0, buf);
+          const char* wb = smem + wl0 + cur;
+          int pa[MT];
+#pragma unroll
+          for (int i = 0; i < MT; ++i) pa[i] = boff[i][kw];
+          asm volatile("" : "+v"(f0v), "+v"(f1v));
+#pragma unroll
+          for (int kt = 0; kt < 2; ++kt) {
+            if constexpr (TAIL == 2) {
+              if (kt == 1 && c * 2 + 1 >= p.KTT) break;
+            }
+            if constexpr (NT <= 6) {
+              u32x4 a[NT], b[MT];
+#pragma unroll
+              for (int j = 0; j < NT; ++j) a[j] = *reinterpret_cast<const u32x4*>(wb + (kt * NTB + j) * 1024);
+#pragma unroll
+              for (int i = 0; i < MT; ++i) b[i] = *reinterpret_cast<const u32x4*>(hal + ((pa[i] ^ (kt ? f1v : f0v)) + rowoff));
+#pragma unroll
+              for (int i = 0; i < MT; ++i)
+#pragma unroll
+                for (int j = 0; j < NT; ++j)
+                  acc[i][j] = __builtin_amdgcn_mfma_f32_16x16x32_bf16(*reinterpret_cast<const bf16x8*>(&a[j]),
+                                                                      *reinterpret_cast<const bf16x8*>(&b[i]), acc[i][j], 0, 0, 0);
+            } else {
+              constexpr int GS = (NT + 1) / 2;
+              u32x4 b[MT];
+#pragma unroll
+              for (int i = 0; i < MT; ++i) b[i] = *reinterpret_cast<const u32x4*>(hal + ((pa[i] ^ (kt ? f1v : f0v)) + rowoff));
+#pragma unroll
+              for (int j0 = 0; j0 < NT; j0 += GS) {
+                u32x4 a[GS];
+#pragma unroll
+                for (int j = 0; j < GS; ++j)
+                  if (j0 + j < NT) a[j] = *reinterpret_cast<const u32x4*>(wb + (kt * NTB + j0 + j) * 1024);
+#pragma unroll
+                for (int i = 0; i < MT; ++i)
+#pragma unroll
+                  for (int j = 0; j < GS; ++j)
+                    if (j0 + j < NT)
+                      acc[i][j0 + j] = __builtin_amdgcn_mfma_f32_16x16x32_bf16(*reinterpret_cast<const bf16x8*>(&a[j]),
+                                                                               *reinterpret_cast<const bf16x8*>(&b[i]), acc[i][j0 + j], 0, 0, 0);
+                __builtin_amdgcn_sched_barrier(0);
+              }
+            }
+          }
+          cur ^= WBUF;
+        }
+        rowoff += rowBytes;
+        f0v ^= flip;
+        f1v ^= flip;
+      }
+      if (c + 1 < nChunks) {
+        __syncthreads();
+        stage_halo(c + 1, false);
+        setup_w(c + 1);
+        issue_w(cur);
+      }
     }
   }
   UPA_STAMP_AT(10);
@@ -405,28 +569,30 @@
 #endif
 }
 
-template <int KS, int STRIDE, int WM, int WN, int MT, int NT, int TAIL = 0>
+template <int KS, int STRIDE, int WM, int WN, int MT, int NT, int TAIL = 0, bool OLD = false>
 __global__ __launch_bounds__(512, 4) void conv_big_kernel(const BigParams p) {
-  conv_big_body<KS, STRIDE, WM, WN, MT, NT, TAIL>(p, (int)blockIdx.x);
-}
-
-template <int KS, int STRIDE, int WM, int WN, int MT, int NT, int TAIL = 0>
+  conv_big_body<KS, STRIDE, WM, WN, MT, NT, TAIL, OLD>(p, (int)blockIdx.x);
+}
+
+template <int KS, int STRIDE, int WM, int WN, int MT, int NT, int TAIL = 0, bool OLD = false>
 __global__ __launch_bounds__(512, 4) void conv_big_pair_kernel(const BigParams p0, const BigParams p1, const int split) {
-  if ((int)blockIdx.x < split) conv_big_body<KS, STRIDE, WM, WN, MT, NT, TAIL>(p0, (int)blockIdx.x);
-  else conv_big_body<KS, STRIDE, WM, WN, MT, NT, TAIL>(p1, (int)blockIdx.x - split);
-}
-template <int KS, int STRIDE, int WM, int WN, int MT, int NT, int TAIL = 0>
+  if ((int)blockIdx.x < split) conv_big_body<KS, STRIDE, WM, WN, MT, NT, TAIL, OLD>(p0, (int)blockIdx.x);
+  else conv_big_body<KS, STRIDE, WM, WN, MT, NT, TAIL, OLD>(p1, (int)blockIdx.x - split);
+}
+template <int KS, int STRIDE, int WM, int WN, int MT, int NT, int TAIL = 0, bool OLD = false>
 __global__ __launch_bounds__(512, 4) void conv_big_tri_kernel(const BigParams p0, const BigParams p1, const BigParams p2, const int s0,
                                                               const int s1) {
-  if ((int)blockIdx.x < s0) conv_big_body<KS, STRIDE, WM, WN, MT, NT, TAIL>(p0, (int)blockIdx.x);
-  else if ((int)blockIdx.x < s1) conv_big_body<KS, STRIDE, WM, WN, MT, NT, TAIL>(p1, (int)blockIdx.x - s0);
-  else conv_big_body<KS, STRIDE, WM, WN, MT, NT, TAIL>(p2, (int)blockIdx.x - s1);
-}
-
-template <int KS_, int STRIDE_, int WM_, int WN_, int MT_, int NT_, int TAIL_>
+  if ((int)blockIdx.x < s0) conv_big_body<KS, STRIDE, WM, WN, MT, NT, TAIL, OLD>(p0, (int)blockIdx.x);
+  else if ((int)blockIdx.x < s1) conv_big_body<KS, STRIDE, WM, WN, MT, NT, TAIL, OLD>(p1, (int)blockIdx.x - s0);
+  else conv_big_body<KS, STRIDE, WM, WN, MT, NT, TAIL, OLD>(p2, (int)blockIdx.x - s1);
+}
+
+template <int KS_, int STRIDE_, int WM_, int WN_, int MT_, int NT_, int TAIL_, bool OLD_ = false>
 struct BigCfg {
   static constexpr int NTB = WN_ * NT_;
-  __device__ static __forceinline__ void run(const BigParams& p, int bid) { conv_big_body<KS_, STRIDE_, WM_, WN_, MT_, NT_, TAIL_>(p, bid); }
+  static constexpr bool HOIST = big_hoisted(MT_, NT_);
+  using Old = BigCfg<KS_, STRIDE_, WM_, WN_, MT_, NT_, TAIL_, true>;
+  __device__ static __forceinline__ void run(const BigParams& p, int bid) { conv_big_body<KS_, STRIDE_, WM_, WN_, MT_, NT_, TAIL_, OLD_>(p, bid); }
 };
 template <class CA, class CB>
 __global__ __launch_bounds__(512, 4) void conv_big_mix_kernel(const BigParams a0, const BigParams a1, const BigParams b0, const BigParams b1,
@@ -449,6 +615,13 @@
   p.magicIW = (unsigned)((0x100000000ULL + p.IWp - 1) / p.IWp);
 }
 size_t big_halo_bytes(const BigParams& p) { return (((size_t)p.IH * p.IWp * 8 + 63) & ~(size_t)63) * 16; }
+int big_loop_form(const BigParams& p, int ntb, int bm, const upa_opts* opts) {
+  if (UPA_OPT(opts, conv_big_loop) == 1) return 1;
+  if (!big_hoisted(bm / 128, ntb)) return 1;
+  if (p.KS > 1 && (p.IWp & 3) != 0) return 1;
+  if (((size_t)p.IH * p.W + 2 * (size_t)p.IWp) * (size_t)p.ldx * 2 >= ((size_t)1 << 31)) return 1;
+  return 0;
+}
 
 bool big_pick_tile(BigParams& p, int bm, int ntb, size_t lds_cap) {
   struct Pick { int th, tw, tight; };
@@ -499,52 +672,78 @@
   return best >= 0;
 }
 
-template <int KS, int STRIDE, int WM, int WN, int MT, int NT, int TAIL = 0>
+template <int KS, int STRIDE, int WM, int WN, int MT, int NT, int TAIL = 0, bool OLD = false>
 int big_launch_inst(const BigParams& p, size_t lds, hipStream_t s) {
+  if constexpr (!OLD && !big_hoisted(MT, NT)) return big_launch_inst<KS, STRIDE, WM, WN, MT, NT, TAIL, true>(p, lds, s);
+  else {
+  if constexpr (!OLD) {
+    if (p.loop) return big_launch_inst<KS, STRIDE, WM, WN, MT, NT, TAIL, true>(p, lds, s);
+  }
   constexpr int NTB = WN * NT;
   const dim3 grid((unsigned)((long)p.tilesX * p.tilesY * p.N), (unsigned)cdiv(p.NTn, NTB));
-  auto kern = conv_big_kernel<KS, STRIDE, WM, WN, MT, NT, TAIL>;
-  if (hipError_t e = upa_full_lds<conv_big_kernel<KS, STRIDE, WM, WN, MT, NT, TAIL>>(); e != hipSuccess) {
+  auto kern = conv_big_kernel<KS, STRIDE, WM, WN, MT, NT, TAIL, OLD>;
+  if (hipError_t e = upa_full_lds<conv_big_kernel<KS, STRIDE, WM, WN, MT, NT, TAIL, OLD>>(); e != hipSuccess) {
     upa_set_error("conv_big: cannot raise LDS limit: %s", hipGetErrorString(e));
     return UPA_ELAUNCH;
   }
   hipLaunchKernelGGL(kern, grid, dim3(512), lds, s, p);
   UPA_LAUNCH_CHECK();
   return UPA_OK;
-}
-
-template <int KS, int STRIDE, int WM, int WN, int MT, int NT, int TAIL = 0>
+  }
+}
+
+template <int KS, int STRIDE, int WM, int WN, int MT, int NT, int TAIL = 0, bool OLD = false>
 int big_launch_pair_inst(const BigParams& p0, const BigParams& p1, size_t lds, hipStream_t s) {
+  if constexpr (!OLD && !big_hoisted(MT, NT)) return big_launch_pair_inst<KS, STRIDE, WM, WN, MT, NT, TAIL, true>(p0, p1, lds, s);
+  else {
+  if constexpr (!OLD) {
+    if (p0.loop || p1.loop) return big_launch_pair_inst<KS, STRIDE, WM, WN, MT, NT, TAIL, true>(p0, p1, lds, s);
+  }
   constexpr int NTB = WN * NT;
   const long t0 = (long)p0.tilesX * p0.tilesY * p0.N, t1 = (long)p1.tilesX * p1.tilesY * p1.N;
   if (cdiv(p0.NTn, NTB) != cdiv(p1.NTn, NTB) || t0 + t1 >= (1L << 31)) return UPA_EUNSUPPORTED;
   const dim3 grid((unsigned)(t0 + t1), (unsigned)cdiv(p0.NTn, NTB));
-  if (hipError_t e = upa_full_lds<conv_big_pair_kernel<KS, STRIDE, WM, WN, MT, NT, TAIL>>(); e != hipSuccess) {
+  if (hipError_t e = upa_full_lds<conv_big_pair_kernel<KS, STRIDE, WM, WN, MT, NT, TAIL, OLD>>(); e != hipSuccess) {
     upa_set_error("conv_big: cannot raise LDS limit: %s", hipGetErrorString(e));
     return UPA_ELAUNCH;
   }
-  hipLaunchKernelGGL((conv_big_pair_kernel<KS, STRIDE, WM, WN, MT, NT, TAIL>), grid, dim3(512), lds, s, p0, p1, (int)t0);
+  hipLaunchKernelGGL((conv_big_pair_kernel<KS, STRIDE, WM, WN, MT, NT, TAIL, OLD>), grid, dim3(512), lds, s, p0, p1, (int)t0);
   UPA_LAUNCH_CHECK();
   return UPA_OK;
-}
-
-template <int KS, int STRIDE, int WM, int WN, int MT, int NT, int TAIL = 0>
+  }
+}
+
+template <int KS, int STRIDE, int WM, int WN, int MT, int NT, int TAIL = 0, bool OLD = false>
 int big_launch_tri_inst(const BigParams& p0, const BigParams& p1, const BigParams& p2, size_t lds, hipStream_t s) {
+  if constexpr (!OLD && !big_hoisted(MT, NT)) return big_launch_tri_inst<KS, STRIDE, WM, WN, MT, NT, TAIL, true>(p0, p1, p2, lds, s);
+  else {
+  if constexpr (!OLD) {
+    if (p0.loop || p1.loop || p2.loop) return big_launch_tri_inst<KS, STRIDE, WM, WN, MT, NT, TAIL, true>(p0, p1, p2, lds, s);
+  }
   constexpr int NTB = WN * NT;
   const long t0 = (long)p0.tilesX * p0.tilesY * p0.N, t1 = (long)p1.tilesX * p1.tilesY * p1.N, t2 = (long)p2.tilesX * p2.tilesY * p2.N;
   if (cdiv(p0.NTn, NTB) != cdiv(p1.NTn, NTB) || cdiv(p0.NTn, NTB) != cdiv(p2.NTn, NTB) || t0 + t1 + t2 >= (1L << 31)) return UPA_EUNSUPPORTED;
   const dim3 grid((unsigned)(t0 + t1 + t2), (unsigned)cdiv(p0.NTn, NTB));
-  if (hipError_t e = upa_full_lds<conv_big_tri_kernel<KS, STRIDE, WM, WN, MT, NT, TAIL>>(); e != hipSuccess) {
+  if (hipError_t e = upa_full_lds<conv_big_tri_kernel<KS, STRIDE, WM, WN, MT, NT, TAIL, OLD>>(); e != hipSuccess) {
     upa_set_error("conv_big: cannot raise LDS limit: %s", hipGetErrorString(e));
     return UPA_ELAUNCH;
   }
-  hipLaunchKernelGGL((conv_big_tri_kernel<KS, STRIDE, WM, WN, MT, NT, TAIL>), grid, dim3(512), lds, s, p0, p1, p2, (int)t0, (int)(t0 + t1));
+  hipLaunchKernelGGL((conv_big_tri_kernel<KS, STRIDE, WM, WN, MT, NT, TAIL, OLD>), grid, dim3(512), lds, s, p0, p1, p2, (int)t0, (int)(t0 + t1));
   UPA_LAUNCH_CHECK();
   return UPA_OK;
-}
-
-template <class CA, class CB>
+  }
+}
+
+template <class CA, class CB, bool OLD = false>
 int big_launch_mix(const BigParams* pa, int na, const BigParams* pb, int nb, size_t lds, hipStream_t s) {
+  if constexpr (!OLD && !(CA::HOIST && CB::HOIST)) return big_launch_mix<typename CA::Old, typename CB::Old, true>(pa, na, pb, nb, lds, s);
+  else {
+  if constexpr (!OLD) {
+    bool old = false;
+    for (int i = 0; i < na; ++i) old = old || pa[i].loop;
+    for (int i = 0; i < nb; ++i) old = old || pb[i].loop;
+    if (old) return big_launch_mix<typename CA::Old, typename CB::Old, true>(pa, na, pb, nb, lds, s);
+  }
   long t[4] = {0, 0, 0, 0};
   for (int i = 0; i < na; ++i) { t[i] = (long)pa[i].tilesX * pa[i].tilesY * pa[i].N; if (pa[i].NTn > CA::NTB) return UPA_EUNSUPPORTED; }
   for (int i = 0; i < nb; ++i) { t[2 + i] = (long)pb[i].tilesX * pb[i].tilesY * pb[i].N; if (pb[i].NTn > CB::NTB) return UPA_EUNSUPPORTED; }
@@ -558,6 +757,7 @@
                      (int)t[0], (int)(t[0] + t[1]), (int)(t[0] + t[1] + t[2]));
   UPA_LAUNCH_CHECK();
   return UPA_OK;
+  }
 }
 
 template <int WM, int WN, int MT, int NT>
@@ -632,6 +832,7 @@
   p.tilesX = cdiv(p.OW, p.TW);
   p.tilesY = cdiv(p.OH, p.TH);
   lds = big_halo_bytes(p) + 2 * (size_t)(2 * ntb * 1024) + 256;
+  p.loop = big_loop_form(p, ntb, bm, opts);
   return UPA_OK;
 }
 int branch_tail_launch(const BigParams& p, int kind, int ntb, int bm, size_t lds, hipStream_t s) {
@@ -803,6 +1004,7 @@
   p.tilesY = cdiv(p.OH, p.TH);
   lds = big_halo_bytes(p) + 2 * (size_t)(2 * ntb * 1024) + 256;
   if (lds > 160 * 1024) return UPA_EUNSUPPORTED;
+  p.loop = big_loop_form(p, ntb, bm, opts);
   return UPA_OK;
 }
 template <int WM, int WN, int MT, int NT>
@@ -836,6 +1038,19 @@
   if (variant) *variant = (1 << 23) | (ntb << 4) | (bm >> 7);
   if (query_only || rc != UPA_OK) return rc;
   return big_dispatch(p, ntb, bm, lds, (hipStream_t)stream);
+}
+
+extern "C" int upa_conv_big_loop_form(int n, int h, int w, int cin, int cout, int k, int stride, const upa_opts* opts) {
+  UPA_CHECK_ARG(n > 0 && h > 0 && w > 0 && cin > 0 && cout > 0 && k >= 1 && k <= 3 && (stride == 1 || stride == 2), "conv_big_loop_form: bad args");
+  BigParams p;
+  memset(&p, 0, sizeof(p));
+  p.N = n; p.H = h; p.W = w; p.Cin = cin; p.ldx = cin; p.Cout = cout; p.ldy = cout;
+  p.KS = k; p.stride = stride; p.pad = k / 2;
+  p.OH = (h + 2 * p.pad - k) / stride + 1; p.OW = (w + 2 * p.pad - k) / stride + 1;
+  int ntb = 0, bm = 0;
+  size_t lds = 0;
+  if (const int rc = big_prepare(p, ntb, bm, lds, opts, false); rc != UPA_OK) return rc;
+  return p.loop;
 }
 
 int upa_conv_big_launch_interleave(BigParams p, void* stream, const upa_opts* opts) {
diff --git a/ultralytics_pro_amd/csrc/conv_pipe.h b/ultralytics_pro_amd/csrc/conv_pipe.h
--- a/ultralytics_pro_amd/csrc/conv_pipe.h
+++ b/ultralytics_pro_amd/csrc/conv_pipe.h
@@ -66,6 +66,7 @@
   float* stats;
   int stats_ld;
   int il_h, il_w, il_c;
+  int loop;
 };
 bool upa_conv_big_eligible(const ConvShape& s, const upa_opts* opts);
 int upa_conv_big_launch(BigParams p, int query_only, int* variant, void* stream, const upa_opts* opts);
```

New measurement: 60580. 1.1% lower.
